# TissueImageAnalytics/cerberus

Measured on AMD Instinct MI355X. Metric: Mpx/sec WSI tiled inference (all heads), higher is better.
Workload: dtype f32

## Files before the change

### cerberus_amd/csrc/cerb_api.hip

```cpp
#include "cerb_net.h"

static thread_local std::string g_err;
int cerb_set_error(const std::string& m) {
    g_err = m;
    return 1;
}
extern "C" int cerb_version(void) { return 1; }
extern "C" const char* cerb_last_error(void) { return g_err.c_str(); }
std::atomic<long long> g_devbuf_bytes{0};
extern "C" size_t cerb_device_bytes_held(void) { const long long v = g_devbuf_bytes.load(); return v > 0 ? (size_t)v : 0; }
thread_local hipStream_t g_call_stream = nullptr;

static int alloc_dev(cerb_net* net, size_t bytes, void** out) {
    if (net->reusing) {
        if (net->reuse_cursor >= net->n_finalize_allocs || net->dev_alloc_bytes[net->reuse_cursor] != bytes)
            return fail("reload: the tensors do not have the shapes the handle was finalized with");
        *out = net->dev_allocs[net->reuse_cursor++];
        return 0;
    }
    void* d = nullptr;
    HIP_OK(hipMalloc(&d, bytes));
    net->dev_allocs.push_back(d);
    net->dev_alloc_bytes.push_back(bytes);
    *out = d;
// ... 366 lines not shown
        }
        for (int di : net->dense_idx) {
            const DecoderCfg& d = net->dec[di];
            const std::string p = "output_head." + d.name + "." + d.head + ".x";
            const HostTensor *w1, *b1, *w2, *b2;
            Fold f;
            if (get(net, p + ".0.block.0.conv.weight", {96, 64, 1, 1}, &w1) || get(net, p + ".0.block.0.conv.bias", {96}, &b1) ||
                bn_fold(net, p + ".0.block.0.bn", 96, &f) || get(net, p + ".1.conv.weight", {d.out_ch, 96, 1, 1}, &w2) ||
                get(net, p + ".1.conv.bias", {d.out_ch}, &b2))
                return 1;
            std::vector<float> w1p(6 * 4 * 64 * 4), b1p(96), w2p(6 * 64 * 4, 0.f), b2p(32, 0.f);
            for (int blk = 0; blk < 6; ++blk)
                for (int G = 0; G < 4; ++G)
                    for (int lane = 0; lane < 64; ++lane)
                        for (int t = 0; t < 4; ++t) {
                            const int hid = blk * 16 + (lane & 15), ci = G * 16 + 4 * (lane >> 4) + t;
                            w1p[((blk * 4 + G) * 64 + lane) * 4 + t] = w1->data[(size_t)hid * 64 + ci] * f.scale[hid];
                        }
            for (int c = 0; c < 96; ++c) b1p[c] = b1->data[c] * f.scale[c] + f.shift[c];
            for (int blk = 0; blk < 6; ++blk)
                for (int lane = 0; lane < 64; ++lane)
                    for (int r = 0; r < 4; ++r) {
                        const int o = lane & 15, hid = blk * 16 + 4 * (lane >> 4) + r;
                        w2p[(blk * 64 + lane) * 4 + r] = (o < d.out_ch) ? w2->data[(size_t)o * 96 + hid] : 0.f;
                    }
            for (int c = 0; c < d.out_ch; ++c) b2p[c] = b2->data[c];
            std::vector<float> w2q(2 * 24 * 64, 0.f);
            for (int set = 0; set < 2; ++set)
                for (int blk = 0; blk < 6; ++blk)
                    for (int r = 0; r < 4; ++r)
                        for (int lane = 0; lane < 64; ++lane) {
                            const int o = 4 * set + (lane & 3), hid = blk * 16 + 4 * (lane >> 4) + r;
                            if (o < d.out_ch) w2q[((set * 6 + blk) * 64 + lane) * 4 + r] = w2->data[(size_t)o * 96 + hid];
                        }
            if (!net->fold_bn) {
                float *r1, *rb1, *r2, *rb2;
                if (upload(net, w1->data, &r1) || upload(net, b1->data, &rb1) || upload(net, w2->data, &r2) || upload(net, b2->data, &rb2)) return 1;
                net->head_rw1.push_back(r1); net->head_rb1.push_back(rb1); net->head_rw2.push_back(r2); net->head_rb2.push_back(rb2);
                net->param_slots[p + ".0.block.0.conv.weight"].push_back({r1, 96 * 64});
                net->param_slots[p + ".0.block.0.conv.bias"].push_back({rb1, 96});
                net->param_slots[p + ".1.conv.weight"].push_back({r2, (long long)d.out_ch * 96});
                net->param_slots[p + ".1.conv.bias"].push_back({rb2, d.out_ch});
                if (store_bn(net, "head." + std::to_string(net->head_rw1.size() - 1), {p + ".0.block.0.bn"}, 96)) return 1;
            }
            float *dw1, *db1, *dw2, *db2;
            float* dw2q;
            if (upload(net, w1p, &dw1) || upload(net, b1p, &db1) || upload(net, w2p, &dw2) || upload(net, b2p, &db2) || upload(net, w2q, &dw2q)) return 1;
            net->head_w1.push_back(dw1); net->head_b1.push_back(db1); net->head_w2.push_back(dw2); net->head_b2.push_back(db2); net->head_w2q.push_back(dw2q);
        }
    }
    if (net->pc_idx >= 0) {
        const int oc = net->dec[net->pc_idx].out_ch;
        const std::string p = "decoder_head.Patch-Class";
        Fold f1, f2;
        const HostTensor *w1, *b1, *w2, *b2;
        if (bn_fold(net, p + ".bn1", 512, &f1) || bn_fold(net, p + ".bn2", 256, &f2) || get(net, p + ".conv1.weight", {256, 512, 1, 1}, &w1) ||
            get(net, p + ".conv1.bias", {256}, &b1) || get(net, p + ".conv2.weight", {oc, 256, 1, 1}, &w2) || get(net, p + ".conv2.bias", {oc}, &b2))
            return 1;
        if (!net->fold_bn) {
            if (upload(net, w1->data, &net->pc_rw1) || upload(net, b1->data, &net->pc_rb1) || upload(net, w2->data, &net->pc_rw2) ||
                upload(net, b2->data, &net->pc_rb2) || store_bn(net, "pc.bn1", {p + ".bn1"}, 512) || store_bn(net, "pc.bn2", {p + ".bn2"}, 256))
                return 1;
            net->param_slots[p + ".conv1.weight"].push_back({net->pc_rw1, 256 * 512});
            net->param_slots[p + ".conv1.bias"].push_back({net->pc_rb1, 256});
            net->param_slots[p + ".conv2.weight"].push_back({net->pc_rw2, (long long)oc * 256});
            net->param_slots[p + ".conv2.bias"].push_back({net->pc_rb2, oc});
        }
        std::vector<float> w1t(512 * 256), b1f(256), w2t(256 * 16, 0.f), b2f(16, 0.f);
        for (int o = 0; o < 256; ++o) {
            for (int c = 0; c < 512; ++c) w1t[(size_t)c * 256 + o] = w1->data[(size_t)o * 512 + c] * f2.scale[o];
            b1f[o] = b1->data[o] * f2.scale[o] + f2.shift[o];
        }
        for (int o = 0; o < oc; ++o) {
            for (int c = 0; c < 256; ++c) w2t[(size_t)c * 16 + o] = w2->data[(size_t)o * 256 + c];
            b2f[o] = b2->data[o];
        }
        if (upload(net, f1.scale, &net->pc_bn1s) || upload(net, f1.shift, &net->pc_bn1b) || upload(net, w1t, &net->pc_w1t) ||
            upload(net, b1f, &net->pc_b1) || upload(net, w2t, &net->pc_w2t) || upload(net, b2f, &net->pc_b2))
            return 1;
    }
    if (!net->fold_bn) {
        std::vector<float> z(512, 0.f);
        if (upload(net, z, &net->zero_bias)) return 1;
    }
    if (!net->fold_bn) HIP_OK(hipDeviceSynchronize());
    if (net->reusing && net->reuse_cursor != net->n_finalize_allocs) return fail("reload: fewer tensors than the handle was finalized with");
    if (!net->reusing) net->n_finalize_allocs = net->dev_allocs.size();
    net->reusing = false;
    net->host.clear();
    net->finalized = true;
    return 0;
}

int prof_begin(cerb_net* net, const std::string& name, const std::string& kernel, double flops, hipStream_t st) {
    if (!net->profiling) return 0;
    if (net->prof_n == net->prof.size()) {
        cerb_net::ProfRec r;
        HIP_OK(hipEventCreate(&r.e0));
        HIP_OK(hipEventCreate(&r.e1));
        net->prof.push_back(r);
    }
    cerb_net::ProfRec& r = net->prof[net->prof_n];
    r.name = name; r.kernel = kernel; r.flops = flops;
    HIP_OK(hipEventRecord(r.e0, st));
    net->prof_open = true;
    return 0;
}
int prof_end(cerb_net* net, hipStream_t st) {
    if (!net->profiling) return 0;
    HIP_OK(hipEventRecord(net->prof[net->prof_n].e1, st));
    net->prof_n++;
    net->prof_open = false;
    return 0;
}

int train_wino2_fresh(cerb_net* net, const std::string& name, PackedConv& cm, int dgrad, hipStream_t st) {
    if (net->fold_bn) return 0;
    bool& used = dgrad ? cm.wino_dgrad_used : cm.wino_used;
    bool& stale = dgrad ? cm.wino_dgrad_stale : cm.wino_stale;
    used = true;
    if (!stale) return 0;
    auto rit = net->raw.find(name);
    if (rit == net->raw.end()) return fail("conv " + name + ": no raw weights to re-pack");
    const size_t nw = (size_t)cm.cout * cm.cin * 9, nu = (size_t)cm.cout * cm.cin * 16;
    for (int g = 0; g < cm.groups; ++g)
        HIP_OK(cerb_launch_pack_wino(rit->second.w + g * nw, (dgrad ? cm.wino_dgrad : cm.wino) + g * nu, dgrad ? cm.cin : cm.cout, dgrad ? cm.cout : cm.cin, dgrad, st));
    stale = false;
    return 0;
}

int train_wino4_slot(cerb_net* net, const std::string& name, PackedConv& cm, int w4b, int dgrad, hipStream_t st, float** out) {
    float*& slot = cm.wino4_t[w4b][dgrad];
    if (!slot) {
        auto rit = net->raw.find(name);
        if (rit == net->raw.end()) return fail("conv " + name + ": no raw weights for the F(4x4) transform");
        const size_t nw = (size_t)cm.cout * cm.cin * 9, nu = (size_t)cm.cout * cm.cin * 36;
        void* d = nullptr;
        HIP_OK(hipMalloc(&d, (size_t)cm.groups * nu * 4));
        net->dev_allocs.push_back(d);
        net->dev_alloc_bytes.push_back((size_t)cm.groups * nu * 4);
        slot = (float*)d;
        (void)nw;
        HIP_OK(cerb_launch_pack_wino4(rit->second.w, slot, dgrad ? cm.cin : cm.cout, dgrad ? cm.cout : cm.cin, dgrad, w4b, cm.groups, st));
    }
    *out = slot;
    return 0;
}

static constexpr int kPlanarLowest = 0;
static const char* const kPlanarFamily[4] = {"conv_wino4_planar<f4x4,16x16x2,eighth-res>", "conv_wino4_planar<f4x4,16x16x2,quarter-res>",
                                             "conv_wino4p<f4x4,16x16x2,planar,half-res>", "conv_wino4p<f4x4,16x16x2,planar>"};
static const char* const kPlanarEntryFamily[4] = {"upsample2_add_planar<eighth-res>", "upsample2_add_planar<quarter-res>", "upsample2_add_planar", "upsample2_add_planar"};

int run_conv(cerb_net* net, const std::string& name, const float* in, const float* prev, const float* resid, float* out, int N,
             int H, int W, int relu, int mode, long long in_gs, long long prev_gs, hipStream_t st, double* macs,
             const int* roi, long long planar_out_gs) {
    auto it = net->conv.find(name);
    if (it == net->conv.end()) return fail("internal: conv " + name + " not packed");
    const PackedConv& c = it->second;
    struct BnReq {
        cerb_net* n;
        ~BnReq() { n->conv_bn_part = nullptr; }
    } bn_req{net};
    net->conv_bn_bpg = 0;
    ConvParams p;
    memset(&p, 0, sizeof(p));
    p.in = in; p.prev = prev; p.wpack = c.w; p.bias = c.b; p.resid = resid; p.out = out;
    p.N = N; p.H = H; p.W = W; p.Cin = c.cin; p.Cout = c.cout;
    p.Ho = (c.stride == 2) ? H / 2 : H;
    p.Wo = (c.stride == 2) ? W / 2 : W;
    p.relu = relu;
    p.groups = c.groups;
    p.in_gs = in_gs; p.prev_gs = prev_gs;
    p.w_gs = (long long)c.cout * c.cin * c.ks * c.ks;
    p.bias_gs = c.cout;
    p.resid_gs = 0;
    p.out_gs = (long long)N * p.Ho * p.Wo * c.cout;
    p.pk_off = net->packed_items ? 0 : 1;
    if (macs) {
        *macs += (double)c.groups * N * p.Ho * p.Wo * (double)c.cout * c.cin * c.ks * c.ks;
        if (!out) return 0;
    }
    const double fl = 2.0 * (double)c.groups * N * p.Ho * p.Wo * (double)c.cout * c.cin * c.ks * c.ks;
    const long long map_px = (long long)p.Ho * p.Wo;
    const bool use_w4 = net->conv_algo == 5 || net->conv_algo == 7 || (net->conv_algo == 6 && map_px >= 256);
    const bool planar = planar_out_gs > 0;
    static const long long w4b_max_px = [] {
        const char* e = cerb_dev_getenv("CERB_W4B_MAX_PX");
        return e ? atoll(e) : 4096ll;
    }();
    const bool w4b = !planar && (net->conv_algo == 7 || (net->conv_algo == 6 && map_px <= w4b_max_px)) && c.cin % 64 == 0;
    if (planar && !(use_w4 && c.wino && mode == 0 && net->fold_bn && !resid)) return fail("internal: conv " + name + " cannot take the planar path");
    if (use_w4 && c.wino && mode == 0 && (!it->second.host_w.empty() || !net->fold_bn)) {
        PackedConv& cm = it->second;
        float* train_slot = nullptr;
        if (!net->fold_bn && train_wino4_slot(net, name, cm, w4b ? 1 : 0, 0, st, &train_slot)) return 1;
        float*& slot4 = !net->fold_bn ? train_slot : (w4b ? cm.wino4b : cm.wino4);
        if (!slot4) {
            std::vector<float> w4;
            for (int g = 0; g < cm.groups; ++g) pack_wino4(cm.host_w.data() + (size_t)g * cm.cout * cm.cin * 9, cm.cout, cm.cin, &w4, w4b ? 1 : 0);
            void* d = nullptr;
            HIP_OK(hipMalloc(&d, w4.size() * 4));
            net->dev_allocs.push_back(d);
            net->dev_alloc_bytes.push_back(w4.size() * 4);
            HIP_OK(hipMemcpy(d, w4.data(), w4.size() * 4, hipMemcpyHostToDevice));
            slot4 = (float*)d;
        }
        p.wpack = slot4;
        p.w_gs = (long long)c.cout * c.cin * 36;
        double fl_done = fl;
        if (roi && roi[1] > roi[0] && roi[3] > roi[2]) {
            p.roi_y0 = roi[0]; p.roi_y1 = roi[1]; p.roi_x0 = roi[2]; p.roi_x1 = roi[3];
            const double ty = (roi[1] + 15) / 16 - roi[0] / 16, tx = (roi[3] + 15) / 16 - roi[2] / 16;
            fl_done = fl * (ty * 16.0 * tx * 16.0) / ((double)p.Ho * p.Wo);
        }
        if (planar) {
            p.out_gs = planar_out_gs;
            p.level_tag = net->planar_level == 3 ? 1 : net->planar_level == 2 ? 0 : 2;
            p.pl_byp = cerb_planar_blocks(p.Ho);
            p.pl_bxp = cerb_planar_blocks(p.Wo);
        }
        if (prof_begin(net, name, planar ? kPlanarFamily[net->planar_level & 3] : w4b ? (cerb_wino4b_packed(p) ? (resid ? "conv_wino4b<f4x4,16t,res>" : "conv_wino4b<f4x4,16t>") : (resid ? "conv_wino4b<f4x4,16x16,res>" : "conv_wino4b<f4x4,16x16>")) : (resid ? "conv_wino4<f4x4,16x16x2,res>" : "conv_wino4<f4x4,16x16x2>"), fl_done, st)) return 1;
        if (net->conv_bn_part && !planar && !resid && !(roi && roi[1] > roi[0] && roi[3] > roi[2])) {
            p.bn_part = net->conv_bn_part;
            net->conv_bn_bpg = w4b ? cerb_wino4b_bn_blocks(p) : N * ((p.Ho + 15) / 16) * ((p.Wo + 15) / 16);
        }
        HIP_OK(planar ? cerb_launch_wino4p(p, st) : w4b ? cerb_launch_wino4b(p, st) : cerb_launch_wino4(p, st));
        if (prof_end(net, st)) return 1;
        return 0;
    }
    if (net->conv_algo && c.wino && mode == 0) {
        if (train_wino2_fresh(net, name, it->second, 0, st)) return 1;
        p.wpack = c.wino;
        p.w_gs = (long long)c.cout * c.cin * 16;
        double fl_done = fl;
        if (roi && roi[1] > roi[0] && roi[3] > roi[2]) {
            p.roi_y0 = roi[0]; p.roi_y1 = roi[1]; p.roi_x0 = roi[2]; p.roi_x1 = roi[3];
            const double ty = (roi[1] + 7) / 8 - roi[0] / 8, tx = (roi[3] + 15) / 16 - roi[2] / 16;
            fl_done = fl * (ty * 8.0 * tx * 16.0) / ((double)p.Ho * p.Wo);
        }
        if (prof_begin(net, name, resid ? "conv_wino<f2x2,8x16,res>" : "conv_wino<f2x2,8x16>", fl_done, st)) return 1;
        HIP_OK(cerb_launch_wino(p, st));
        if (prof_end(net, st)) return 1;
        return 0;
    }
    const std::string kn = "conv_igemm<ks" + std::to_string(c.ks) + ",s" + std::to_string(c.stride) + ",mode" + std::to_string(mode) +
                           (p.Wo < 32 ? ",16x16>" : ",8x32>");
    if (prof_begin(net, name, kn, fl, st)) return 1;
    HIP_OK(cerb_launch_conv(p, c.ks, c.stride, mode, st));
    if (prof_end(net, st)) return 1;
    return 0;
}

static int forward_impl(cerb_net* net, const cerb_forward_io* io, hipStream_t st, double* macs) {
    g_call_stream = st;
    const bool dry = (macs != nullptr) && (io->tiles == nullptr) && (io->tiles_f32 == nullptr);
    const int N = io->n, H = io->h, W = io->w;
    if (N <= 0 || H <= 0 || W <= 0 || (H % 16) || (W % 16)) return fail("cerb_net_forward: tile H,W must be positive multiples of 16");
    const int out_h = io->out_h > 0 ? io->out_h : H, out_w = io->out_w > 0 ? io->out_w : W;
    if (out_h > H || out_w > W) return fail("cerb_net_forward: crop larger than tile");
    const int hs[5] = {H, H / 2, H / 4, H / 8, H / 16}, ws[5] = {W, W / 2, W / 4, W / 8, W / 16};
    const size_t D = net->trunk_idx.size();
    const size_t guard = cerb_conv_guard_bytes(W);
    const int planar_lowest = [] {
        const char* e = cerb_dev_getenv("CERB_PLANAR_LOWEST");
        return e ? atoi(e) : kPlanarLowest;
    }();
    auto level_is_planar = [&](int u) {
        if (dry || !net->planar || !net->fold_bn || net->conv_algo != 6 || net->head_algo < 1) return false;
        for (int v = 3; v >= u; --v) {
            if (v < planar_lowest) return false;
            auto c0 = net->conv.find("dec." + std::to_string(v) + ".0"), c1 = net->conv.find("dec." + std::to_string(v) + ".1");
            if (c0 == net->conv.end() || c1 == net->conv.end() || !c0->second.wino || !c1->second.wino) return false;
            const long long px = (long long)hs[3 - v] * ws[3 - v];
            if ((hs[3 - v] & 3) || (ws[3 - v] & 3)) return false;
            const bool ok = v >= 2 ? px >= 4096 && c0->second.cin == 64 && c0->second.cout == 64 && c1->second.cout == 64
                                   : px >= 256 && c0->second.cin % 16 == 0 && c0->second.cout % 64 == 0 && c1->second.cin == c0->second.cout && c1->second.cout % 64 == 0;
            if (!ok) return false;
        }
        return true;
    };
    if (!dry) {
        if (net->x0.ensure((size_t)N * H * W * 64 * 4, guard) || net->pool.ensure((size_t)N * hs[1] * ws[1] * 64 * 4, guard)) return fail_alloc();
        for (int i = 1; i < 5; ++i)
            if (net->x[i].ensure((size_t)N * hs[i] * ws[i] * kFilters[i] * 4, guard)) return fail_alloc();
        if (net->ta.ensure((size_t)N * hs[1] * ws[1] * 64 * 4, guard) || net->tb.ensure((size_t)N * hs[1] * ws[1] * 64 * 4, guard) ||
            net->cm.ensure((size_t)N * hs[4] * ws[4] * 256 * 4, guard))
            return fail_alloc();
        if (D) {
            static const bool exact_ws = cerb_dev_getenv("CERB_LEGACY_WS") == nullptr;
            size_t need_sum = 0, need_mid = 0;
            const int oc[4] = {128, 64, 64, 64};
            for (int u = 0; u < 4; ++u) {
                if (exact_ws && level_is_planar(u)) continue;
                const std::string n0 = "dec." + std::to_string(u) + ".0";
                auto c0 = net->conv.find(n0);
                const size_t px = (size_t)D * N * hs[3 - u] * ws[3 - u];
                need_sum = std::max(need_sum, px * (size_t)(c0 != net->conv.end() ? c0->second.cin : 256) * 4);
                need_mid = std::max(need_mid, px * (size_t)(c0 != net->conv.end() ? c0->second.cout : 256) * 4);
            }
            if (!exact_ws) need_sum = need_mid = D * (size_t)N * H * W * 64 * 4;
            if (net->dmid.ensure(need_mid, guard)) return fail_alloc();
            if (net->conv_algo && net->dsum.ensure(need_sum, guard)) return fail_alloc();
            for (int u = 0; u < 4; ++u) {
                if (exact_ws && level_is_planar(u)) continue;
                if (net->dout[u].ensure(D * (size_t)N * hs[3 - u] * ws[3 - u] * oc[u] * 4, guard)) return fail_alloc();
            }
        }
    }
    if (macs) *macs += (double)N * H * W * 64.0 * 147.0;
    if (!dry) {
        StemParams sp;
        sp.tiles = io->tiles; sp.tiles_f32 = io->tiles ? nullptr : io->tiles_f32; sp.wpack = net->stem_w; sp.bias = net->stem_b; sp.out = net->x0.p; sp.N = N; sp.H = H; sp.W = W; sp.relu = 1;
        sp.tiles_x = sp.tiles_y = 0;
        if (prof_begin(net, "stem", "stem_conv7x7", 2.0 * N * H * W * 64.0 * 147.0, st)) return 1;
        HIP_OK(cerb_launch_stem(sp, st));
        if (prof_end(net, st)) return 1;
        if (prof_begin(net, "maxpool", "maxpool3x3s2", 0.0, st)) return 1;
        HIP_OK(cerb_launch_maxpool(net->x0.p, net->pool.p, N, H, W, 64, st));
        if (prof_end(net, st)) return 1;
    }
    float* cur = dry ? nullptr : net->pool.p;
    int inpl = 64;
    for (int li = 0; li < 4; ++li) {
        const int planes = kFilters[li + 1];
        const int Hi = (li == 0) ? hs[1] : hs[li], Wi = (li == 0) ? ws[1] : ws[li];
        for (int b = 0; b < kLayers[li]; ++b) {
            const std::string p = "backbone.layer" + std::to_string(li + 1) + "." + std::to_string(b);
            const int stride = (b == 0 && li > 0) ? 2 : 1;
            const int hin = (b == 0) ? Hi : hs[li + 1], win = (b == 0) ? Wi : ws[li + 1];
            float* t1 = dry ? nullptr : net->ta.p;
            const bool last = (b == kLayers[li] - 1);
            float* outb = dry ? nullptr : (((kLayers[li] - 1 - b) % 2 == 0) ? net->x[li + 1].p : net->tb.p);
            (void)last;
            const float* idt = cur;
            if (run_conv(net, p + ".conv1", cur, nullptr, nullptr, t1, N, hin, win, 1, 0, 0, 0, st, macs)) return 1;
            if (stride != 1 || inpl != planes) {
                float* ds = dry ? nullptr : net->pool.p;
                if (run_conv(net, p + ".downsample", cur, nullptr, nullptr, ds, N, hin, win, 0, 0, 0, 0, st, macs)) return 1;
                idt = ds;
            }
            if (run_conv(net, p + ".conv2", t1, nullptr, idt, outb, N, hs[li + 1], ws[li + 1], 1, 0, 0, 0, st, macs)) return 1;
            cur = outb;
            inpl = planes;
        }
    }
    if (run_conv(net, "conv_map", dry ? nullptr : net->x[4].p, nullptr, nullptr, dry ? nullptr : net->cm.p, N, hs[4], ws[4], 0, 0, 0, 0, st, macs)) return 1;

    const long long tile_stride = io->tile_stride ? io->tile_stride : (long long)out_h * out_w;
    const long long row_stride = io->row_stride ? io->row_stride : out_w;
    if (net->pc_idx >= 0) {
        if (macs) *macs += (double)N * (512.0 * 256 + 256.0 * net->dec[net->pc_idx].out_ch);
        const bool want = io->out && io->out[net->pc_idx];
        const bool wantl = io->logits && io->logits[net->pc_idx];
        if (!dry && (want || wantl)) {
            PatchClassParams pp;
            memset(&pp, 0, sizeof(pp));
            pp.x4 = net->x[4].p; pp.bn1_s = net->pc_bn1s; pp.bn1_b = net->pc_bn1b; pp.w1t = net->pc_w1t; pp.b1 = net->pc_b1;
            pp.w2t = net->pc_w2t; pp.b2 = net->pc_b2;
            pp.N = N; pp.Hf = hs[4]; pp.Wf = ws[4]; pp.out_ch = net->dec[net->pc_idx].out_ch;
            pp.out_h = out_h; pp.out_w = out_w;
            pp.logits = wantl ? io->logits[net->pc_idx] : nullptr;
            pp.out = want ? (float*)io->out[net->pc_idx] : nullptr;
            pp.tile_off = io->tile_off; pp.tile_stride = tile_stride; pp.row_stride = row_stride;
            if (prof_begin(net, "patch_class", "patch_class", 2.0 * N * (512.0 * 256 + 256.0 * pp.out_ch), st)) return 1;
            HIP_OK(cerb_launch_patch_class(pp, st));
            if (prof_end(net, st)) return 1;
        }
    }
    if (D) {
        const float* skips[4] = {dry ? nullptr : net->x[3].p, dry ? nullptr : net->x[2].p, dry ? nullptr : net->x[1].p, dry ? nullptr : net->x0.p};
        const float* prev = dry ? nullptr : net->cm.p;
        long long prev_gs = 0;
        const int oc[4] = {128, 64, 64, 64};
        int roi_out[4][4], roi_mid[4][4], roi_sum[4][4];
        const bool any_logits = [&] {
            if (!io->logits) return false;
            for (size_t k = 0; k < net->dec.size(); ++k)
                if (io->logits[k]) return true;
            return false;
        }();
        const bool use_roi = !dry && net->crop_roi && (net->conv_algo == 1 || net->conv_algo >= 5) && !any_logits && (out_h < H || out_w < W);
        if (use_roi) {
            int y0 = (int)((H - out_h) * 0.5), x0 = (int)((W - out_w) * 0.5), y1 = y0 + out_h, x1 = x0 + out_w;
            for (int u = 3; u >= 0; --u) {
                const int hh = hs[3 - u], ww = ws[3 - u];
                auto widen = [&](int* r, const int* in, int d) {
                    r[0] = std::max(0, (in[0] - d) & ~3); r[1] = std::min(hh, (in[1] + d + 3) & ~3);
                    r[2] = std::max(0, (in[2] - d) & ~3); r[3] = std::min(ww, (in[3] + d + 3) & ~3);
                };
                const int win[4] = {y0, y1, x0, x1};
                widen(roi_out[u], win, 0);
                widen(roi_mid[u], roi_out[u], 1);
                widen(roi_sum[u], roi_mid[u], 1);
                y0 = std::max(0, roi_sum[u][0] / 2 - 1); y1 = std::min(hh / 2, (roi_sum[u][1] - 1) / 2 + 2);
                x0 = std::max(0, roi_sum[u][2] / 2 - 1); x1 = std::min(ww / 2, (roi_sum[u][3] - 1) / 2 + 2);
            }
        }
        bool feat_planar = false, prev_planar = false;
        for (int u = 0; u < 4; ++u) {
            const int hh = hs[3 - u], ww = ws[3 - u];
            const std::string n0 = "dec." + std::to_string(u) + ".0", n1 = "dec." + std::to_string(u) + ".1";
            const int cmid = net->conv[n0].cout;
            const int cin0 = net->conv[n0].cin;
            const bool lvl_planar = level_is_planar(u);
            if (lvl_planar) {
                PlanarBuf &bs = u == 3 ? net->psum : u == 2 ? net->psum2 : u == 1 ? net->psum1 : net->psum0;
                PlanarBuf &bm = u == 3 ? net->pmid : u == 2 ? net->pmid2 : u == 1 ? net->pmid1 : net->pmid0;
                const int cout1 = net->conv[n1].cout;
                PlanarBuf& bo = cout1 == cin0 ? bs : u == 1 ? net->pout1 : net->pout0;
                if (bs.ensure((int)D, N, hh, ww, cin0, st) || bm.ensure((int)D, N, hh, ww, cmid, st) || (&bo != &bs && bo.ensure((int)D, N, hh, ww, cout1, st)))
                    return fail_alloc();
                if (prof_begin(net, n0 + ".up", kPlanarEntryFamily[u], 0.0, st)) return 1;
                HIP_OK(cerb_launch_upsample2_add_planar(skips[u], prev, bs.b.p, (int)D, N, hh, ww, cin0, prev_gs, bs.gs(), use_roi ? roi_sum[u] : nullptr, prev_planar ? 1 : 0, st));
                if (prof_end(net, st)) return 1;
                net->planar_level = u;
                if (run_conv(net, n0, bs.b.p, nullptr, nullptr, bm.b.p, N, hh, ww, 1, 0, bs.gs(), 0, st, macs, use_roi ? roi_mid[u] : nullptr, bm.gs()))
                    return 1;
                if (run_conv(net, n1, bm.b.p, nullptr, nullptr, bo.b.p, N, hh, ww, 1, 0, bm.gs(), 0, st, macs, use_roi ? roi_out[u] : nullptr, bo.gs()))
                    return 1;
                if (u == 3) feat_planar = true;
                prev = bo.b.p;
                prev_gs = bo.gs();
                prev_planar = true;
                continue;
            }
            if (prev_planar) return fail("internal: a tile-planar decoder level feeds an NHWC one");
            if (net->conv_algo && net->conv[n0].wino && !dry) {
                if (prof_begin(net, n0 + ".up", "upsample2_add", 0.0, st)) return 1;
                HIP_OK(cerb_launch_upsample2_add(skips[u], prev, net->dsum.p, (int)D, N, hh, ww, cin0, prev_gs, use_roi ? roi_sum[u] : nullptr, st));
                if (prof_end(net, st)) return 1;
                if (run_conv(net, n0, net->dsum.p, nullptr, nullptr, net->dmid.p, N, hh, ww, 1, 0, (long long)N * hh * ww * cin0, 0, st, macs,
                             use_roi ? roi_mid[u] : nullptr))
                    return 1;
            } else if (run_conv(net, n0, skips[u], prev, nullptr, dry ? nullptr : net->dmid.p, N, hh, ww, 1, 1, 0, prev_gs, st, macs)) return 1;
            if (run_conv(net, n1, dry ? nullptr : net->dmid.p, nullptr, nullptr, dry ? nullptr : net->dout[u].p, N, hh, ww, 1, 0,
                         (long long)N * hh * ww * cmid, 0, st, macs, use_roi ? roi_out[u] : nullptr))
                return 1;
            prev = dry ? nullptr : net->dout[u].p;
            prev_gs = (long long)N * hh * ww * oc[u];
        }
        HeadParams hps[8];
        int n_hp = 0;
        double head_flops = 0.0;
        for (size_t k = 0; k < net->dense_idx.size(); ++k) {
            const int di = net->dense_idx[k];
            const size_t tk = (size_t)net->trunk_of[k];
            const DecoderCfg& d = net->dec[di];
            if (macs) *macs += (double)N * H * W * (64.0 * 96 + 96.0 * d.out_ch);
            const bool want = io->out && io->out[di];
            const bool wantl = io->logits && io->logits[di];
            if (dry || !(want || wantl)) continue;
            HeadParams hp;
            memset(&hp, 0, sizeof(hp));
            hp.feat = feat_planar ? net->psum.b.p + tk * net->psum.gs() : net->dout[3].p + tk * (size_t)N * H * W * 64;
            hp.feat_planar = feat_planar ? 1 : 0;
            hp.pl_byp = cerb_planar_blocks(H);
            hp.pl_bxp = cerb_planar_blocks(W);
            hp.w1p = net->head_w1[k]; hp.b1 = net->head_b1[k]; hp.w2p = net->head_w2[k]; hp.b2 = net->head_b2[k]; hp.w2q = net->head_w2q[k];
            hp.N = N; hp.H = H; hp.W = W; hp.out_ch = d.out_ch; hp.kind = d.kind;
            hp.crop_y0 = (int)((H - out_h) * 0.5); hp.crop_x0 = (int)((W - out_w) * 0.5);
            hp.out_h = want ? out_h : 0; hp.out_w = want ? out_w : 0;
            hp.roi = use_roi ? 1 : 0;
            hp.logits = wantl ? io->logits[di] : nullptr;
            hp.absmax_bits = io->logit_absmax ? io->logit_absmax + di : nullptr;
            if (want) {
                if (d.kind == 0) hp.out_inst = (float*)io->out[di];
                else if (io->type_is_u8) hp.out_type_u8 = (unsigned char*)io->out[di];
                else hp.out_type_i64 = (long long*)io->out[di];
            }
            hp.tile_off = io->tile_off; hp.tile_stride = tile_stride; hp.row_stride = row_stride;
            const double head_px = hp.roi ? (double)out_h * (((hp.crop_x0 + out_w + 15) / 16 - hp.crop_x0 / 16) * 16.0) : (double)H * W;
            const double fl = 2.0 * N * head_px * (64.0 * 96 + 96.0 * d.out_ch);
            if (net->head_algo == 0) {
                if (prof_begin(net, "head." + d.name, "head", fl, st)) return 1;
                HIP_OK(cerb_launch_head(hp, st));
                if (prof_end(net, st)) return 1;
            } else {
                if (n_hp == 8) {
// ... 231 lines not shown
```

### cerberus_amd/csrc/cerb_net.h

```cpp
#ifndef CERB_NET_H
#define CERB_NET_H
#include <hip/hip_runtime.h>

#include <algorithm>
#include <cmath>
#include <cstdio>
#include <cstdlib>
#include <cstring>
#include <map>
#include <atomic>
#include <string>
#include <vector>

#include "../../include/cerberus_hip.h"
#include "cerb_common.h"

hipError_t cerb_launch_conv(const ConvParams& p, int ks, int stride, int mode, hipStream_t st);
hipError_t cerb_launch_wino(ConvParams p, hipStream_t st);
hipError_t cerb_launch_wino4(ConvParams p, hipStream_t st);
hipError_t cerb_launch_wino4b(ConvParams p, hipStream_t st);
int cerb_wino4b_bn_blocks(const ConvParams& p);
bool cerb_wino4b_packed(const ConvParams& p);
hipError_t cerb_launch_wino4p(ConvParams p, hipStream_t st);
hipError_t cerb_launch_upsample2_add_planar(const float* skip, const float* prev, float* out, int groups, int N, int H, int W, int C, long long prev_gs,
                                            long long out_gs, const int* roi, int prev_planar, hipStream_t st);
hipError_t cerb_launch_upsample2_add(const float* skip, const float* prev, float* out, int groups, int N, int H, int W, int C,
                                     long long prev_gs, const int* roi, hipStream_t st);
extern "C" int cerb_conv_chunk(int ks, int stride);
struct StemParams {
    const unsigned char* tiles;
    const float* tiles_f32;
    const float* wpack;
    const float* bias;
    float* out;
    int N, H, W, tiles_x, tiles_y;
    int relu;
};
hipError_t cerb_launch_stem(StemParams p, hipStream_t st);
size_t cerb_bn_workspace_bytes(int groups, long long rows, int C);
hipError_t cerb_launch_bn_stats(const float* x, long long group_stride, long long rows, int C, int groups, float eps, float* mean, float* rstd,
                                float* var_unbiased, void* ws, hipStream_t st);
hipError_t cerb_launch_bn_apply(float* x, const float* src, const float* resid, long long group_stride, long long rows, int C, int groups, const float* mean,
                                const float* rstd, const float* gamma, const float* beta, int relu, hipStream_t st);
hipError_t cerb_launch_bn_finalize(const double* partial, int blocks, long long rows, int C, float eps, float* mean, float* rstd, float* var_unbiased, hipStream_t st,
                                   int groups = 1, void* fold_ws = nullptr);
size_t cerb_bn_fold_workspace_bytes(int groups, int C);
hipError_t cerb_launch_pointwise(const float* in, const float* w, const float* bias, float* out, long long rows, int cin, int cout, const float* in_scale,
                                 hipStream_t st, double* bn_part = nullptr, int* bn_blocks = nullptr);
hipError_t cerb_launch_crop_gap(const float* x, int N, int H, int W, int C, int y0, int ch, int x0, int cw, float* out, hipStream_t st);
hipError_t cerb_launch_copy_multi(int count, float* const* dst, const float* const* src, const long long* n, void** dev_tab, size_t* dev_bytes,
                                  std::vector<char>* host_prev, hipStream_t st);
hipError_t cerb_launch_bn_bwd(const float* dz, const float* z, const float* y, float* dy, float* dresid, long long group_stride, long long rows, int C, int groups,
                              const float* mean, const float* rstd, const float* gamma, const float* beta, float* dgamma, float* dbeta, int relu, int dy_assign, void* ws, hipStream_t st, unsigned long long eval_mask = 0, int dresid_assign = 0,
                              const double* pre_part = nullptr, int pre_bpg = 0);
int cerb_head_bwd2_blocks();
hipError_t cerb_launch_conv_bwd(const float* x, const float* dy, const float* w, float* dx, float* dw, float* db, int G, int N, int H, int W, int Cin, int Cout,
                                int ks, int stride, long long x_gs, hipStream_t st);
hipError_t cerb_launch_stem_wgrad(const unsigned char* tiles, const float* dy, float* dw, int N, int H, int W, hipStream_t st);
hipError_t cerb_launch_maxpool_bwd(const float* x, const float* ypool, const float* dy, float* dx, int N, int H, int W, int C, hipStream_t st);
hipError_t cerb_launch_maxpool_idx(const float* in, float* out, unsigned* idx, int N, int H, int W, int C, hipStream_t st);
hipError_t cerb_launch_maxpool_bwd_idx(const unsigned* idx, const float* dy, float* dx, int N, int H, int W, int C, hipStream_t st);
bool cerb_upadd_bwd_fused_ok(int H, int W, int C, int G);
hipError_t cerb_launch_upadd_bwd(const float* dout, float* dskip, float* dprev, int G, int N, int H, int W, int C, long long prev_gs, int shared_prev, hipStream_t st,
                                 unsigned group_mask = 0xffffffffu, int skip_assign = 0, int prev_assign = 0);
hipError_t cerb_launch_pointwise_bwd(const float* x, const float* dy, const float* w, float* dx, float* dw, float* db, long long rows, int cin, int cout,
                                     const float* in_scale, int dx_assign, hipStream_t st);
hipError_t cerb_launch_crop_gap_bwd(const float* dg, float* dx, int N, int H, int W, int C, int y0, int ch, int x0, int cw, hipStream_t st);
hipError_t cerb_launch_adam(float* p, const float* g, float* m, float* v, long long n, float lr, float b1, float b2, float eps, int step, hipStream_t st);
size_t cerb_wgrad_workspace_bytes(int G, int N, int Ho, int Wo, int Cin, int Cout, int ks, int* slices_out);
size_t cerb_stem_wgrad_workspace_bytes();
hipError_t cerb_launch_pack_stem(const float* w_raw, float* out, hipStream_t st);
struct PackJob {
    const float* w;
    float* out;
    long long total;
    int cout, cin, kind, a, b, pad;
};
hipError_t cerb_launch_pack_multi(const PackJob* jobs, int count, void** dev_tab, size_t* dev_bytes, std::vector<char>* host_prev, hipStream_t st);
hipError_t cerb_launch_adam_multi(int count, float* const* p, const float* const* g, float* const* m, float* const* v, const long long* n, float lr, float b1,
                                  float b2, float eps, int step, hipStream_t st);
hipError_t cerb_launch_pack_conv(const float* w_raw, float* out, int cout, int cin, int ks, int chunk, hipStream_t st);
hipError_t cerb_launch_pack_wino(const float* w_raw, float* out, int cout, int cin, int dgrad, hipStream_t st);
hipError_t cerb_launch_pack_wino4(const float* w_raw, float* out, int cout, int cin, int dgrad, int chunk32, int groups, hipStream_t st);
hipError_t cerb_launch_dilate2(const float* dy, float* d, long long n, int H, int W, int C, hipStream_t st);
size_t cerb_pw_wgrad_small_workspace_bytes(long long rows, int cin, int cout);
hipError_t cerb_launch_pw_wgrad_small(const float* x, const float* dy, float* dw, long long rows, int cin, int cout, void* ws, hipStream_t st);
size_t cerb_pw_bwd_small_workspace_bytes(long long rows, int cin, int cout);
hipError_t cerb_launch_pw_bwd_small(const float* x, const float* dy, const float* w, float* dx, float* dw, float* db, long long rows, int cin, int cout,
                                    int dx_assign, void* ws, hipStream_t st);
hipError_t cerb_launch_stem_wgrad_mfma(const unsigned char* tiles, const float* dy, float* dw, int N, int H, int W, void* ws, hipStream_t st);
hipError_t cerb_launch_colsum(const float* d, long long group_stride, long long rows, int C, int G, float* out, void* ws, hipStream_t st);
bool cerb_wgrad_wino_supported(int H, int W, int Cin, int Cout);
size_t cerb_wgrad_wino_workspace_bytes(int G, int N, int H, int W, int Cin, int Cout);
hipError_t cerb_launch_wgrad_wino(const float* x, const float* dy, float* dw, int G, int N, int H, int W, int Cin, int Cout, long long x_gs, void* ws, hipStream_t st,
                                  float* db);
hipError_t cerb_launch_wgrad(const float* x, const float* dy, float* dw, int G, int N, int H, int W, int Cin, int Cout, int ks, int stride, long long x_gs, void* ws,
                             hipStream_t st, float* db = nullptr);
bool cerb_head_train_supported(long long rows, int cin, int chid, int out);
hipError_t cerb_launch_head_fwd1(const float* prev, const float* w1, const float* b1, float* hid, long long rows, double* bn_part, int* bn_blocks, hipStream_t st,
                                 const float* const* in_bn = nullptr);
hipError_t cerb_launch_head_fwd2(const float* hid, const float* mean, const float* rstd, const float* gamma, const float* beta, const float* w2, const float* b2,
                                 float* logits, long long rows, int out, hipStream_t st);
size_t cerb_head_bwd_workspace_bytes(long long rows, int out);
hipError_t cerb_launch_head_bwd1(const float* hid, const float* dlog, const float* mean, const float* rstd, const float* gamma, const float* beta, const float* w2,
                                 float* dw2, float* db2, float* dgamma, float* dbeta, long long rows, int out, void* ws, hipStream_t st);
hipError_t cerb_launch_head_bwd2(const float* hid, const float* dlog, const float* prev, const float* mean, const float* rstd, const float* gamma, const float* beta,
                                 const float* dgamma, const float* dbeta, const float* w1, const float* w2, float* dprev, float* dw1, float* db1, long long rows, int out,
                                 int eval_mode, int assign, void* ws, hipStream_t st, const float* const* in_bn = nullptr, double* in_part = nullptr);
hipError_t cerb_launch_maxpool(const float* in, float* out, int N, int H, int W, int C, hipStream_t st);
hipError_t cerb_launch_head(const HeadParams& p, hipStream_t st);
hipError_t cerb_launch_head_group(const HeadParams* heads, int n_heads, hipStream_t st, int w2_44);
struct PatchClassParams {
    const float* x4;
    const float* bn1_s;
    const float* bn1_b;
    const float* w1t;
    const float* b1;
    const float* w2t;
    const float* b2;
    int N, Hf, Wf, out_ch;
    int out_h, out_w;
    float* logits;
    float* out;
    const long long* tile_off;
    long long tile_stride, row_stride;
};
hipError_t cerb_launch_patch_class(const PatchClassParams& p, hipStream_t st);

int cerb_set_error(const std::string& m);
static inline int fail(const std::string& m) { return cerb_set_error(m); }
static inline int fail_alloc() { return cerb_set_error("workspace allocation failed") + 1; }
#define HIP_OK(expr)                                                                              \
    do {                                                                                          \
        hipError_t e_ = (expr);                                                                   \
        if (e_ != hipSuccess) return fail(std::string(#expr) + ": " + hipGetErrorString(e_));     \
    } while (0)

struct HostTensor {
    std::vector<int64_t> shape;
    std::vector<float> data;
};

extern "C" size_t cerb_conv_guard_bytes(int tile_w);
extern thread_local hipStream_t g_call_stream;
extern std::atomic<long long> g_devbuf_bytes;
struct DevBuf {
    float* p = nullptr;
    char* raw = nullptr;
    size_t bytes = 0, guard = 0, held = 0;
    int ensure(size_t need, size_t g) {
        if (need <= bytes && g <= guard) return 0;
        release();
        if (hipMalloc(&raw, need + 2 * g) != hipSuccess) {
            raw = nullptr;
            return 1;
        }
        g_devbuf_bytes += (long long)(need + 2 * g);
        held = need + 2 * g;
        if (hipMemsetAsync(raw, 0, need + 2 * g, g_call_stream) != hipSuccess) return 1;
        p = reinterpret_cast<float*>(raw + g);
        bytes = need;
        guard = g;
        return 0;
    }
    void release() {
        if (raw) {
            (void)hipFree(raw);
            g_devbuf_bytes -= (long long)held;
        }
        held = 0;
        raw = nullptr;
        p = nullptr;
        bytes = guard = 0;
    }
};

struct PlanarBuf {
    DevBuf b;
    int h = 0, w = 0, c = 0, groups = 0;
    long long cap_n = 0;
    long long per_image() const { return cerb_planar_elems(1, h, w, c); }
    long long gs() const { return cap_n * per_image(); }
    int ensure(int G, int N, int H, int W, int C, hipStream_t st) {
        if (H == h && W == w && C == c && G == groups && N <= cap_n) return 0;
        const size_t need = (size_t)G * (size_t)N * (size_t)cerb_planar_elems(1, H, W, C) * 4;
        if (need > b.bytes) {
            if (b.ensure(need, 0)) return 1;
        } else if (hipMemsetAsync(b.raw, 0, b.bytes + 2 * b.guard, st) != hipSuccess) {
            return 1;
        }
        h = H; w = W; c = C; groups = G;
        cap_n = (long long)(b.bytes / ((size_t)G * (size_t)cerb_planar_elems(1, H, W, C) * 4));
        return 0;
    }
    void release() { b.release(); h = w = c = groups = 0; cap_n = 0; }
};

struct PackedConv {
    int cin = 0, cout = 0, ks = 0, stride = 1, groups = 1;
    float* w = nullptr;
    float* wino = nullptr;
    float* wino_dgrad = nullptr;
    bool wino_used = false, wino_dgrad_used = false, wino_stale = false, wino_dgrad_stale = false;
    float* wino4_t[2][2] = {{nullptr, nullptr}, {nullptr, nullptr}};
    float* wino4b = nullptr;
    float* wino4 = nullptr;
    std::vector<float> host_w;
    float* b = nullptr;
};

struct DecoderCfg {
    std::string name, head;
    int out_ch = 0;
    int kind = 0;
};

struct cerb_net {
    std::vector<DecoderCfg> dec;
    std::vector<int> dense_idx;
    std::vector<int> trunk_idx;
    std::vector<int> trunk_of;
    int pc_idx = -1;
    std::map<std::string, HostTensor> host;
    bool finalized = false;
    float *stem_w = nullptr, *stem_b = nullptr;
    std::map<std::string, PackedConv> conv;
    std::vector<float*> head_w1, head_b1, head_w2, head_b2, head_w2q;
    float *pc_bn1s = nullptr, *pc_bn1b = nullptr, *pc_w1t = nullptr, *pc_b1 = nullptr, *pc_w2t = nullptr, *pc_b2 = nullptr;
    std::vector<void*> dev_allocs;
    std::vector<size_t> dev_alloc_bytes;
    size_t n_finalize_allocs = 0, reuse_cursor = 0;
    bool reusing = false;
    int fold_bn = 1;
    struct BnDev {
        float *gamma = nullptr, *beta = nullptr;
        int C = 0, groups = 1;
        float *run_mean = nullptr, *run_rstd = nullptr;
        std::vector<char> eval;
    };
    std::map<std::string, BnDev> bn;
    std::vector<float*> head_rw1, head_rb1, head_rw2, head_rb2;
    float *pc_rw1 = nullptr, *pc_rb1 = nullptr, *pc_rw2 = nullptr, *pc_rb2 = nullptr;
    DevBuf t_mean, t_rstd, t_ws, t_hid, t_gap, t_pc1, t_idn, t_dil;
    struct RawW { float* w = nullptr; float* b = nullptr; std::vector<std::string> wkeys, bkeys, bnkeys; };
    std::map<std::string, RawW> raw;
    struct ParamSlot { float* dst; long long n; };
    std::map<std::string, std::vector<ParamSlot>> param_slots;
    float* stem_raw = nullptr;
    std::vector<DevBuf> tape;
    size_t tape_pos = 0;
    void* copy_tab = nullptr;
    size_t copy_tab_bytes = 0;
    std::vector<char> copy_tab_host;
    void* pack_tab = nullptr;
    size_t pack_tab_bytes = 0;
    std::vector<char> pack_tab_host;
    float* zero_bias = nullptr;
    std::map<std::string, std::pair<float*, long long>> grads;
    std::map<std::string, std::vector<std::string>> bn_keys;
    DevBuf x0, pool, x[5], ta, tb, cm, dmid, dsum, dout[4];
    PlanarBuf psum, pmid, pout;
    int planar_level = 3;
    PlanarBuf psum2, pmid2, pout2;
    PlanarBuf psum1, pmid1, pout1, psum0, pmid0, pout0;
    int packed_items = 1;
    int planar = 1;
    bool profiling = false;
    int crop_roi = 1;
    int head_algo = 1;
    int conv_algo = 6;
    struct ProfRec { std::string name, kernel; double flops; hipEvent_t e0, e1; };
    std::vector<ProfRec> prof;
    size_t prof_n = 0;
    bool prof_open = false;
    double* conv_bn_part = nullptr;
    int conv_bn_bpg = 0;
    hipStream_t side = nullptr;
    hipEvent_t ev_fork = nullptr, ev_join = nullptr;
    DevBuf t_ws2;
    ~cerb_net() {
        if (side) { (void)hipStreamSynchronize(side); (void)hipStreamDestroy(side); }
        if (ev_fork) (void)hipEventDestroy(ev_fork);
        if (ev_join) (void)hipEventDestroy(ev_join);
        t_ws2.release();
        for (auto& r : prof) { (void)hipEventDestroy(r.e0); (void)hipEventDestroy(r.e1); }
        for (void* p : dev_allocs) (void)hipFree(p);
        if (copy_tab) (void)hipFree(copy_tab);
        if (pack_tab) (void)hipFree(pack_tab);
        x0.release(); pool.release(); ta.release(); tb.release(); cm.release(); dmid.release(); dsum.release(); psum.release(); pmid.release(); pout.release(); psum2.release(); pmid2.release(); pout2.release(); psum1.release(); pmid1.release(); pout1.release(); psum0.release(); pmid0.release(); pout0.release();
        t_mean.release(); t_rstd.release(); t_ws.release(); t_hid.release(); t_gap.release(); t_pc1.release(); t_idn.release(); t_dil.release();
        for (auto& b : tape) b.release();
        for (auto& b : x) b.release();
        for (auto& b : dout) b.release();
    }
};


static const int kLayers[4] = {3, 4, 6, 3};
static const int kFilters[5] = {64, 64, 128, 256, 512};
int prof_begin(cerb_net* net, const std::string& name, const std::string& kernel, double flops, hipStream_t st);
int prof_end(cerb_net* net, hipStream_t st);
int train_wino2_fresh(cerb_net* net, const std::string& name, PackedConv& cm, int dgrad, hipStream_t st);
int train_wino4_slot(cerb_net* net, const std::string& name, PackedConv& cm, int w4b, int dgrad, hipStream_t st, float** out);
int run_conv(cerb_net* net, const std::string& name, const float* in, const float* prev, const float* resid, float* out, int N, int H, int W, int relu, int mode,
             long long in_gs, long long prev_gs, hipStream_t st, double* macs, const int* roi = nullptr, long long planar_out_gs = 0);
#endif
```

### cerberus_amd/csrc/conv_igemm.hip

```cpp
#include "wino_common.h"

__device__ __forceinline__ f32x4 splat4(float x) {
    f32x4 r = {x, x, x, x};
    return r;
}

template <int KS, int STRIDE, int TH, int TW, int CB, int MODE>
struct ConvCfg {
    static constexpr int PAD = KS / 2;
    static constexpr int GSTEP = (KS == 1) ? STRIDE : 1;
    static constexpr int LSTEP = (KS == 1) ? 1 : STRIDE;
    static constexpr int IH = (KS == 1) ? TH : (TH - 1) * STRIDE + KS;
    static constexpr int IW = (KS == 1) ? TW : (TW - 1) * STRIDE + KS;
    static constexpr int PS = CB + 4;
    static constexpr int NG = CB / 8;
    static constexpr int T = KS * KS;
    static constexpr int NQ = T * NG;
    static constexpr int PARTS = CB / 4;
    static constexpr int PPS = 256 / PARTS;
    static constexpr int NF = IH * IW * PARTS;
    static constexpr int RPS = 32 / TW;
    static constexpr int NM = (IH + RPS - 1) / RPS;
    static constexpr int NE = (2 * IH * 8 + 255) / 256;
    static constexpr int ITER = (MODE == 1) ? NM + NE : (NF + 255) / 256;
    static constexpr int MAIN_FLOATS = IH * IW * PS;
    static constexpr int AR = TH / 2 + 2, AC = TW / 2 + 2;
    static constexpr int NA = AR * AC * PARTS;
    static constexpr int AITER = (NA + 255) / 256;
    static constexpr int AUX_FLOATS = (MODE == 1) ? AR * AC * PS : 0;
    static constexpr int LDS_FLOATS = MAIN_FLOATS + AUX_FLOATS;
    static constexpr int LDS_BYTES = LDS_FLOATS * 4;
    static constexpr int S_PREV = ITER;
    static constexpr int S_BAR = ITER + AITER + 6;
    static constexpr int S_COMB = S_BAR + 1;
    static constexpr int WD = (MODE == 0 && STRIDE == 1) ? 3 : 2;
};

struct Item {
    int g, cb, n, oy0, ox0, tx, ty;
};

template <int KS, int STRIDE, int TH, int TW, int CB, int MODE>
__global__ __launch_bounds__(256, 2) void conv_igemm_kernel(ConvParams p) {
    using C = ConvCfg<KS, STRIDE, TH, TW, CB, MODE>;
    constexpr int WD = C::WD;
    static_assert(TH * TW == 256, "tile must hold 256 pixels (4 waves x 2 x 32)");
    static_assert(MODE == 0 || (KS == 3 && STRIDE == 1 && CB == 32 && C::IH % C::RPS == 0 && C::S_COMB + C::ITER <= C::NQ),
                  "MODE 1 schedule must fit in one chunk");
    static_assert(C::ITER <= 2 * C::NQ || KS == 1, "every staging slice needs a step");
    extern __shared__ __attribute__((aligned(16))) float lds[];

    const int tid = threadIdx.x;
    const int lane = tid & 63;
    const int wave = tid >> 6;
    const int j = lane & 31;
    const int h = lane >> 5;

    const int ncb = p.Cout >> 6;
    const int ntile = p.N * p.tiles_y * p.tiles_x;
    const int per_group = ntile * ncb;
    const int total = per_group * p.groups;
    const int nchunk = p.Cin / CB;
    const int lb = xcd_remap(blockIdx.x, gridDim.x);
    const int base_cnt = total / (int)gridDim.x, rem_cnt = total % (int)gridDim.x;
    int item = lb * base_cnt + min(lb, rem_cnt);
    const int item_end = item + base_cnt + (lb < rem_cnt ? 1 : 0);
    if (item >= item_end) return;

    auto decode = [&](int it) {
        Item w;
        w.g = it / per_group;
        int L = it - w.g * per_group;
        w.cb = L % ncb;
        int t_ = L / ncb;
        w.tx = t_ % p.tiles_x;
        t_ /= p.tiles_x;
        w.ty = t_ % p.tiles_y;
        w.n = t_ / p.tiles_y;
        w.oy0 = w.ty * TH;
        w.ox0 = w.tx * TW;
        return w;
    };
    auto advance = [&](Item w) {
        if (++w.cb == ncb) {
            w.cb = 0;
            if (++w.tx == p.tiles_x) {
                w.tx = 0;
                if (++w.ty == p.tiles_y) {
                    w.ty = 0;
                    if (++w.n == p.N) {
                        w.n = 0;
                        ++w.g;
                    }
                }
            }
        }
        w.oy0 = w.ty * TH;
        w.ox0 = w.tx * TW;
        return w;
    };
    auto in_base = [&](const Item& w) {
        return reinterpret_cast<const char*>(p.in + w.g * p.in_gs) +
               ((((long long)w.n * p.H + (w.oy0 * STRIDE - C::PAD)) * p.W + (w.ox0 * STRIDE - C::PAD)) * p.Cin) * 4;
    };
    auto w_base = [&](const Item& w) {
        return reinterpret_cast<const char*>(p.wpack + w.g * p.w_gs + (long long)w.cb * nchunk * C::NQ * 2 * 256);
    };
    auto touches_border = [&](const Item& w) {
        const int y0 = w.oy0 * STRIDE - C::PAD, x0 = w.ox0 * STRIDE - C::PAD;
        return y0 < 0 || x0 < 0 || y0 + (C::IH - 1) * C::GSTEP + 1 > p.H || x0 + (C::IW - 1) * C::GSTEP + 1 > p.W;
    };

    constexpr int RPS = C::RPS, NM = C::NM, NE = C::NE;
    unsigned soff[MODE == 1 ? 1 + NE : C::ITER];
    int ldsw0, ldswE = 0;
    bool e_last_ok = true;
    const int rowb = p.W * p.Cin * 4;
    if (MODE == 1) {
        const int mrow = (tid >> 3) / TW, mcol = (tid >> 3) % TW, part = tid & 7;
        soff[0] = (unsigned)(((mrow * p.W + mcol) * p.Cin + part * 4) * 4);
        ldsw0 = (mrow * C::IW + mcol) * C::PS + part * 4;
        const int e_iy = tid >> 4, e_ix = TW + ((tid >> 3) & 1);
#pragma unroll
        for (int k = 0; k < NE; ++k) {
            const int iy = min(e_iy + 16 * k, C::IH - 1);
            soff[1 + k] = (unsigned)(((iy * p.W + e_ix) * p.Cin + part * 4) * 4);
        }
        ldswE = (e_iy * C::IW + e_ix) * C::PS + part * 4;
        e_last_ok = e_iy + 16 * (NE - 1) < C::IH;
    } else {
#pragma unroll
        for (int s = 0; s < C::ITER; ++s) {
            const int f = min(tid + s * 256, C::NF - 1);
            const int pix = f / C::PARTS, part = f % C::PARTS;
            soff[s] = (unsigned)((((pix / C::IW) * C::GSTEP * p.W + (pix % C::IW) * C::GSTEP) * p.Cin + part * 4) * 4);
        }
        ldsw0 = (tid / C::PARTS) * C::PS + (tid % C::PARTS) * 4;
    }
    const unsigned wlane = (unsigned)lane * 16u;
    int ldsb[2];
    unsigned ooff[2];
#pragma unroll
    for (int q = 0; q < 2; ++q) {
        const int pl = (wave * 2 + q) * 32 + j;
        const int py = pl / TW, px = pl % TW;
        ldsb[q] = ((py * C::LSTEP) * C::IW + px * C::LSTEP) * C::PS + 4 * h;
        ooff[q] = (unsigned)(((py * p.Wo + px) * p.Cout + 4 * h) * 4);
    }
    float* aux = lds + C::MAIN_FLOATS;
    int aoffM = 0, aoffE[NE];
    float wM[4] = {0.f, 0.f, 0.f, 0.f}, wE[4] = {0.f, 0.f, 0.f, 0.f};
    int auxw0 = 0;
    if (MODE == 1) {
        const int mrow = (tid >> 3) / TW, mcol = (tid >> 3) % TW, part = tid & 7;
        aoffM = (mcol >> 1) * C::PS + part * 4;
        const float lxM = (mcol & 1) ? 0.75f : 0.25f;
        const float lyM = (RPS == 2 && (mrow & 1)) ? 0.75f : 0.25f;
        wM[0] = (1.f - lyM) * (1.f - lxM), wM[1] = (1.f - lyM) * lxM, wM[2] = lyM * (1.f - lxM), wM[3] = lyM * lxM;
        const int e_iy = tid >> 4, e_b = (tid >> 3) & 1;
#pragma unroll
        for (int k = 0; k < NE; ++k) aoffE[k] = ((min(e_iy + 16 * k, C::IH - 1) >> 1) * C::AC + TW / 2) * C::PS + part * 4;
        const float lxE = e_b ? 0.75f : 0.25f, lyE = (e_iy & 1) ? 0.75f : 0.25f;
        wE[0] = (1.f - lyE) * (1.f - lxE), wE[1] = (1.f - lyE) * lxE, wE[2] = lyE * (1.f - lxE), wE[3] = lyE * lxE;
        auxw0 = (tid / C::PARTS) * C::PS + (tid % C::PARTS) * 4;
    }

    f32x4 v[C::ITER];
    f32x4 pvv[C::AITER > 0 ? C::AITER : 1];
    unsigned poff[MODE == 1 ? C::AITER : 1];

    auto issue = [&](__amdgpu_buffer_rsrc_t r, int chunk_off, int s) {
        if (MODE == 1) {
            if (s < NM) v[s] = buf_load(r, soff[0], chunk_off + s * RPS * rowb);
            else v[s] = buf_load(r, soff[1 + s - NM], chunk_off);
        } else {
            v[s] = buf_load(r, soff[s], chunk_off);
        }
    };
    auto prev_offsets = [&](const Item& w) {
        const int Hp = p.H >> 1, Wp = p.W >> 1;
#pragma unroll
        for (int k = 0; k < C::AITER; ++k) {
            const int f = min(tid + k * 256, C::NA - 1);
            const int apix = f / C::PARTS, part = f % C::PARTS;
            const int py = min(max((w.oy0 >> 1) - 1 + apix / C::AC, 0), Hp - 1), px = min(max((w.ox0 >> 1) - 1 + apix % C::AC, 0), Wp - 1);
            poff[k] = (unsigned)(((py * Wp + px) * p.Cin + part * 4) * 4);
        }
    };
    auto prev_base = [&](const Item& w) {
        return reinterpret_cast<const char*>(p.prev + w.g * p.prev_gs + (long long)w.n * (p.H >> 1) * (p.W >> 1) * p.Cin);
    };
    auto write_prev = [&]() {
#pragma unroll
        for (int k = 0; k < C::AITER; ++k)
            if (tid + k * 256 < C::NA) *reinterpret_cast<f32x4*>(aux + auxw0 + k * C::PPS * C::PS) = pvv[k];
    };
    auto combine = [&](int s) {
        const bool main = s < NM;
        const float* a = main ? aux + aoffM + ((s * RPS) >> 1) * C::AC * C::PS : aux + aoffE[main ? 0 : s - NM];
        const f32x4 p00 = *reinterpret_cast<const f32x4*>(a);
        const f32x4 p01 = *reinterpret_cast<const f32x4*>(a + C::PS);
        const f32x4 p10 = *reinterpret_cast<const f32x4*>(a + C::AC * C::PS);
        const f32x4 p11 = *reinterpret_cast<const f32x4*>(a + C::AC * C::PS + C::PS);
        const bool swap = main && RPS == 1 && (s & 1);
        const float* wt = main ? wM : wE;
        f32x4 r = v[s];
        r = __builtin_elementwise_fma(splat4(wt[swap ? 2 : 0]), p00, r);
        r = __builtin_elementwise_fma(splat4(wt[swap ? 3 : 1]), p01, r);
        r = __builtin_elementwise_fma(splat4(wt[swap ? 0 : 2]), p10, r);
        r = __builtin_elementwise_fma(splat4(wt[swap ? 1 : 3]), p11, r);
        v[s] = r;
    };
    auto slice_iy = [&](int s) { return MODE == 1 ? (s < NM ? s * RPS + (tid >> 3) / TW : (tid >> 4) + 16 * (s - NM)) : ((tid + s * 256) / C::PARTS) / C::IW; };
    auto slice_ix = [&](int s) { return MODE == 1 ? (s < NM ? (tid >> 3) % TW : TW + ((tid >> 3) & 1)) : ((tid + s * 256) / C::PARTS) % C::IW; };
    auto slice_ptr = [&](int s) { return MODE == 1 ? (s < NM ? lds + ldsw0 + s * RPS * C::IW * C::PS : lds + ldswE + (s - NM) * 16 * C::IW * C::PS) : lds + ldsw0 + s * C::PPS * C::PS; };
    auto slice_live = [&](int s) { return MODE == 1 ? (s < C::ITER - 1 || e_last_ok) : (tid + s * 256 < C::NF); };
    auto write_tile = [&](const Item& w, bool masked) {
        if (!masked) {
#pragma unroll
            for (int s = 0; s < C::ITER; ++s)
                if (slice_live(s)) *reinterpret_cast<f32x4*>(slice_ptr(s)) = v[s];
        } else {
#pragma unroll
            for (int s = 0; s < C::ITER; ++s) {
                const int gy = w.oy0 * STRIDE - C::PAD + slice_iy(s) * C::GSTEP, gx = w.ox0 * STRIDE - C::PAD + slice_ix(s) * C::GSTEP;
                const bool ok = gy >= 0 && gy < p.H && gx >= 0 && gx < p.W;
                const f32x4 z = {0.f, 0.f, 0.f, 0.f};
                if (slice_live(s)) *reinterpret_cast<f32x4*>(slice_ptr(s)) = ok ? v[s] : z;
            }
        }
    };

    Item w = decode(item);
    {
        const __amdgpu_buffer_rsrc_t r0 = make_rsrc(in_base(w));
#pragma unroll
        for (int s = 0; s < C::ITER; ++s) issue(r0, 0, s);
    }
    if (MODE == 1) {
        prev_offsets(w);
        const __amdgpu_buffer_rsrc_t rp = make_rsrc(prev_base(w));
#pragma unroll
        for (int k = 0; k < C::AITER; ++k) pvv[k] = buf_load(rp, poff[k], 0);
        write_prev();
        __syncthreads();
#pragma unroll
        for (int s = 0; s < C::ITER; ++s) combine(s);
    }
    __amdgpu_buffer_rsrc_t rw = make_rsrc(w_base(w));
    f32x4 wq[WD + 1][2];
#pragma unroll
    for (int d = 0; d < WD; ++d)
#pragma unroll
        for (int s = 0; s < 2; ++s) wq[d][s] = buf_load(rw, wlane, (d * 2 + s) * 1024);

    for (;;) {
        f32x16 acc[2][2];
#pragma unroll
        for (int s = 0; s < 2; ++s)
#pragma unroll
            for (int q = 0; q < 2; ++q)
#pragma unroll
                for (int r = 0; r < 16; ++r) acc[s][q][r] = 0.f;

        const bool more_items = item + 1 < item_end;
        const Item wnx = more_items ? advance(w) : w;
        const __amdgpu_buffer_rsrc_t rw_nx = more_items ? make_rsrc(w_base(wnx)) : rw;
        const bool mask_cur = touches_border(w);

        for (int ch = 0; ch < nchunk; ++ch) {
            __syncthreads();
            write_tile(w, mask_cur);
            __syncthreads();

            const bool last_ch = (ch == nchunk - 1);
            const Item wp_ = last_ch ? wnx : w;
            const int chp = last_ch ? 0 : ch + 1;
            const __amdgpu_buffer_rsrc_t r_stage = make_rsrc(in_base(wp_));
            const int stage_off = chp * (CB * 4);
            __amdgpu_buffer_rsrc_t r_prev = r_stage;
            if (MODE == 1) {
                r_prev = make_rsrc(prev_base(wp_));
                if (last_ch) prev_offsets(wp_);
            }
            const int wcur_off = ch * (C::NQ * 2048);
            const __amdgpu_buffer_rsrc_t rw_over = last_ch ? rw_nx : rw;
            const int wover_off = last_ch ? 0 : (ch + 1) * (C::NQ * 2048);

            f32x4 b0 = *reinterpret_cast<const f32x4*>(lds + ldsb[0]), b1 = *reinterpret_cast<const f32x4*>(lds + ldsb[1]);
            f32x4 bn0 = b0, bn1 = b1;
#pragma unroll
            for (int tap = 0; tap < C::T; ++tap) {
#pragma unroll
                for (int G = 0; G < C::NG; ++G) {
                    const int q = tap * C::NG + G;
                    {
                        if (q + WD < C::NQ) {
                            wq[WD][0] = buf_load(rw, wlane, wcur_off + ((q + WD) * 2 + 0) * 1024);
                            wq[WD][1] = buf_load(rw, wlane, wcur_off + ((q + WD) * 2 + 1) * 1024);
                        } else {
                            wq[WD][0] = buf_load(rw_over, wlane, wover_off + ((q + WD - C::NQ) * 2 + 0) * 1024);
                            wq[WD][1] = buf_load(rw_over, wlane, wover_off + ((q + WD - C::NQ) * 2 + 1) * 1024);
                        }
                        if (q + 1 < C::NQ) {
                            const int tap1 = (q + 1) / C::NG, G1 = (q + 1) % C::NG;
                            const int toff1 = ((tap1 / KS) * C::IW + (tap1 % KS)) * C::PS + G1 * 8;
                            bn0 = *reinterpret_cast<const f32x4*>(lds + ldsb[0] + toff1);
                            bn1 = *reinterpret_cast<const f32x4*>(lds + ldsb[1] + toff1);
                        }
                    }
#pragma unroll
                    for (int s = q; s < C::ITER; s += C::NQ) issue(r_stage, stage_off, s);
                    if (MODE == 1) {
                        if (q >= C::S_PREV && q < C::S_PREV + C::AITER) pvv[q - C::S_PREV] = buf_load(r_prev, poff[q - C::S_PREV], stage_off);
                        if (q == C::S_BAR) {
                            write_prev();
                            __syncthreads();
                        }
                        if (q >= C::S_COMB && q - C::S_COMB < C::ITER) combine(q - C::S_COMB);
                    }
                    __builtin_amdgcn_sched_barrier(0);
#pragma unroll
                    for (int t = 0; t < 4; ++t) {
                        acc[0][0] = __builtin_amdgcn_mfma_f32_32x32x2f32(wq[0][0][t], b0[t], acc[0][0], 0, 0, 0);
                        acc[1][0] = __builtin_amdgcn_mfma_f32_32x32x2f32(wq[0][1][t], b0[t], acc[1][0], 0, 0, 0);
                        acc[0][1] = __builtin_amdgcn_mfma_f32_32x32x2f32(wq[0][0][t], b1[t], acc[0][1], 0, 0, 0);
                        acc[1][1] = __builtin_amdgcn_mfma_f32_32x32x2f32(wq[0][1][t], b1[t], acc[1][1], 0, 0, 0);
                    }
#pragma unroll
                    for (int d = 0; d < WD; ++d) {
                        wq[d][0] = wq[d + 1][0];
                        wq[d][1] = wq[d + 1][1];
                    }
                    b0 = bn0;
                    b1 = bn1;
                }
            }
        }

        {
            const float* bias = p.bias + w.g * p.bias_gs + w.cb * 64 + h * 4;
            const long long origin = (((long long)w.n * p.Ho + w.oy0) * p.Wo + w.ox0) * p.Cout + w.cb * 64;
            const __amdgpu_buffer_rsrc_t r_out = make_rsrc(p.out + w.g * p.out_gs + origin);
            const __amdgpu_buffer_rsrc_t r_res = make_rsrc(p.resid ? p.resid + w.g * p.resid_gs + origin : p.out);
            const bool has_res = p.resid != nullptr;
            const bool partial = (w.oy0 + TH > p.Ho) || (w.ox0 + TW > p.Wo);
#pragma unroll
            for (int q = 0; q < 2; ++q) {
                if (partial) {
                    const int pl = (wave * 2 + q) * 32 + j;
                    if (w.oy0 + pl / TW >= p.Ho || w.ox0 + pl % TW >= p.Wo) continue;
                }
#pragma unroll
                for (int s = 0; s < 2; ++s) {
#pragma unroll
                    for (int rq = 0; rq < 4; ++rq) {
                        const int co = s * 32 + rq * 8;
                        f32x4 o = {acc[s][q][rq * 4 + 0], acc[s][q][rq * 4 + 1], acc[s][q][rq * 4 + 2], acc[s][q][rq * 4 + 3]};
                        o = o + *reinterpret_cast<const f32x4*>(bias + co);
                        if (has_res) o = o + buf_load(r_res, ooff[q], co * 4);
                        if (p.relu) {
                            o[0] = fmaxf(o[0], 0.f);
                            o[1] = fmaxf(o[1], 0.f);
                            o[2] = fmaxf(o[2], 0.f);
                            o[3] = fmaxf(o[3], 0.f);
                        }
                        buf_store(o, r_out, ooff[q], co * 4);
                    }
                }
            }
        }
        if (!more_items) break;
        ++item;
        w = wnx;
        rw = rw_nx;
    }
}

template <int KS, int STRIDE, int TH, int TW, int CB, int MODE>
static hipError_t launch_cfg(ConvParams p, hipStream_t st) {
    using C = ConvCfg<KS, STRIDE, TH, TW, CB, MODE>;
    p.tiles_x = (p.Wo + TW - 1) / TW;
    p.tiles_y = (p.Ho + TH - 1) / TH;
    const long long items = (long long)p.groups * p.N * p.tiles_x * p.tiles_y * (p.Cout / 64);
    auto kern = conv_igemm_kernel<KS, STRIDE, TH, TW, CB, MODE>;
    static bool attr_done[64] = {};
    if (cerb_attr_needed(attr_done)) {
        hipError_t e = hipFuncSetAttribute(reinterpret_cast<const void*>(kern), hipFuncAttributeMaxDynamicSharedMemorySize, C::LDS_BYTES);
        if (e != hipSuccess) return e;
    }
    const int blocks_per_cu = (C::LDS_BYTES * 2 <= 160 * 1024) ? 2 : 1;
    long long grid = 256ll * blocks_per_cu;
    if (grid > items) grid = items;
    hipLaunchKernelGGL(kern, dim3((unsigned)grid), dim3(256), C::LDS_BYTES, st, p);
    return hipGetLastError();
}

extern "C" int cerb_conv_chunk(int ks, int stride) { return (stride == 2) ? 16 : 32; }

extern "C" size_t cerb_conv_guard_bytes(int tile_w) { return (size_t)17 * (size_t)tile_w * 64 * 4 + (64u << 10); }

hipError_t cerb_launch_conv(const ConvParams& p, int ks, int stride, int mode, hipStream_t st) {
    const bool small = p.Wo < 32;
    if (ks == 3 && stride == 1 && mode == 0) return small ? launch_cfg<3, 1, 16, 16, 32, 0>(p, st) : launch_cfg<3, 1, 8, 32, 32, 0>(p, st);
    if (ks == 3 && stride == 1 && mode == 1) return small ? launch_cfg<3, 1, 16, 16, 32, 1>(p, st) : launch_cfg<3, 1, 8, 32, 32, 1>(p, st);
    if (ks == 3 && stride == 2 && mode == 0) return small ? launch_cfg<3, 2, 16, 16, 16, 0>(p, st) : launch_cfg<3, 2, 8, 32, 16, 0>(p, st);
    if (ks == 1 && stride == 1 && mode == 0) return small ? launch_cfg<1, 1, 16, 16, 32, 0>(p, st) : launch_cfg<1, 1, 8, 32, 32, 0>(p, st);
    if (ks == 1 && stride == 2 && mode == 0) return small ? launch_cfg<1, 2, 16, 16, 16, 0>(p, st) : launch_cfg<1, 2, 8, 32, 16, 0>(p, st);
    return hipErrorInvalidValue;
}
```

### cerberus_amd/csrc/conv_wino4p.hip

```cpp
#include <type_traits>

#include "wino_common.h"

namespace {
constexpr int NPOS = 36;
constexpr int NT = 32;
constexpr int CB = 16;
constexpr int V_FLOATS = NPOS * NT * CB;
constexpr int LDS_BYTES = 2 * V_FLOATS * 4;
constexpr int PLANE_BYTES = 16 * 16 * 16 * 4;
constexpr int NS = NPOS;
constexpr int NPOS_A = 32;
#ifndef P4_RING
#define P4_RING 12
#endif
constexpr int RING = P4_RING;
#ifndef P4_WD
#define P4_WD 8
#endif
constexpr int WD = P4_WD;
#ifndef P4_PRE
#define P4_PRE P4_WD
#endif
constexpr int PRE = P4_PRE;
#ifndef P4_WB
#define P4_WB 1
#endif
constexpr int WB = P4_WB;
#ifndef P4_TQ
#define P4_TQ 22
#endif
constexpr int TQ = P4_TQ;
#ifndef P4_HQ
#define P4_HQ 8
#endif
constexpr int HQ = P4_HQ;
constexpr int halo_r(int k) { return k < 6 ? k : k < 14 ? ((k - 6) & 1 ? 5 : 0) : k - 14; }
constexpr int halo_q(int k) { return k < 6 ? 0 : k < 14 ? 1 + (k - 6) / 2 : 5; }
static_assert(NS % RING == 0 && WD + WB <= RING && NS % WB == 0 && PRE == WD && PRE <= RING, "weight ring");
static_assert(HQ + 10 <= TQ && TQ + 13 < NS && TQ + 8 + 4 <= NS, "the halo must be requested before the transform starts, the interior after its registers are free");
constexpr int BIAS_XI = 7;
constexpr int CHUNK_W_BYTES = NPOS * 4 * 1024;
constexpr int WAVE_W_BYTES = NPOS * 1024;

#ifdef P4_PROF
constexpr int PROF_BYTES = 16 * 40 * 8;
__device__ unsigned long long p4_prof_buf[16 * 40];
#ifndef P4_PROF_WAVE
#define P4_PROF_WAVE 0
#endif
#else
#ifdef P4_ABL_LDSPATCH
constexpr int PROF_BYTES = 16 * 1024;
#else
constexpr int PROF_BYTES = 0;
#endif
#endif

template <int I>
using IC = std::integral_constant<int, I>;
template <int B, int E, class F>
__device__ __forceinline__ void static_for(F&& f) {
    if constexpr (B < E) {
        f(IC<B>{});
        static_for<B + 1, E>(f);
    }
}

#ifndef P4_WAUX
#define P4_WAUX 0
#endif
#ifndef P4_PAUX
#define P4_PAUX 0
#endif

template <bool AGPR, bool ZERO>
__device__ __forceinline__ void mfma_step(f32x4& c0, f32x4& c1, const f32x4& av, const f32x4& b0, const f32x4& b1) {
#define P4_STEP_BODY(FIRST0, FIRST1)                               \
    "v_mfma_f32_16x16x4_f32 %0, %2, %6, " FIRST0 "\n\t"             \
    "v_mfma_f32_16x16x4_f32 %1, %2, %10, " FIRST1 "\n\t"            \
    "v_mfma_f32_16x16x4_f32 %0, %3, %7, %0\n\t"                     \
    "v_mfma_f32_16x16x4_f32 %1, %3, %11, %1\n\t"                    \
    "v_mfma_f32_16x16x4_f32 %0, %4, %8, %0\n\t"                     \
    "v_mfma_f32_16x16x4_f32 %1, %4, %12, %1\n\t"                    \
    "v_mfma_f32_16x16x4_f32 %0, %5, %9, %0\n\t"                     \
    "v_mfma_f32_16x16x4_f32 %1, %5, %13, %1"
#define P4_STEP_IN "v"(av[0]), "v"(av[1]), "v"(av[2]), "v"(av[3]), "v"(b0[0]), "v"(b0[1]), "v"(b0[2]), "v"(b0[3]), "v"(b1[0]), "v"(b1[1]), "v"(b1[2]), "v"(b1[3])
    if constexpr (ZERO) {
        if constexpr (AGPR) asm volatile(P4_STEP_BODY("0", "0") : "=&a"(c0), "=&a"(c1) : P4_STEP_IN);
        else asm volatile(P4_STEP_BODY("0", "0") : "=&v"(c0), "=&v"(c1) : P4_STEP_IN);
    } else {
        if constexpr (AGPR) asm volatile(P4_STEP_BODY("%0", "%1") : "+a"(c0), "+a"(c1) : P4_STEP_IN);
        else asm volatile(P4_STEP_BODY("%0", "%1") : "+v"(c0), "+v"(c1) : P4_STEP_IN);
    }
#undef P4_STEP_BODY
#undef P4_STEP_IN
}
#ifndef P4_ILV
#define P4_ILV 0
#endif
template <bool AGPR, bool ZERO>
__device__ __forceinline__ void mfma_pair(f32x4& c0, f32x4& c1, float a, float b0, float b1) {
    if constexpr (ZERO) {
        if constexpr (AGPR) asm volatile("v_mfma_f32_16x16x4_f32 %0, %2, %3, 0\n\tv_mfma_f32_16x16x4_f32 %1, %2, %4, 0" : "=&a"(c0), "=&a"(c1) : "v"(a), "v"(b0), "v"(b1));
        else asm volatile("v_mfma_f32_16x16x4_f32 %0, %2, %3, 0\n\tv_mfma_f32_16x16x4_f32 %1, %2, %4, 0" : "=&v"(c0), "=&v"(c1) : "v"(a), "v"(b0), "v"(b1));
    } else {
        if constexpr (AGPR) asm volatile("v_mfma_f32_16x16x4_f32 %0, %2, %3, %0\n\tv_mfma_f32_16x16x4_f32 %1, %2, %4, %1" : "+a"(c0), "+a"(c1) : "v"(a), "v"(b0), "v"(b1));
        else asm volatile("v_mfma_f32_16x16x4_f32 %0, %2, %3, %0\n\tv_mfma_f32_16x16x4_f32 %1, %2, %4, %1" : "+v"(c0), "+v"(c1) : "v"(a), "v"(b0), "v"(b1));
    }
}
__device__ __forceinline__ void wait_mfma_results() { asm volatile("s_nop 15\n\ts_nop 3"); }

__device__ __forceinline__ int fresh_lane() {
    int l;
    asm volatile("v_mbcnt_lo_u32_b32 %0, -1, 0\n\tv_mbcnt_hi_u32_b32 %0, -1, %0" : "=v"(l));
    return l;
}

__device__ __forceinline__ f32x4 sub4(const f32x4& x, const f32x4& y) {
    f32x2 lo, hi;
    const f32x2 xl = {x[0], x[1]}, xh = {x[2], x[3]}, yl = {y[0], y[1]}, yh = {y[2], y[3]};
    asm("v_pk_add_f32 %0, %1, %2 neg_lo:[0,1] neg_hi:[0,1]" : "=v"(lo) : "v"(xl), "v"(yl));
    asm("v_pk_add_f32 %0, %1, %2 neg_lo:[0,1] neg_hi:[0,1]" : "=v"(hi) : "v"(xh), "v"(yh));
    return f32x4{lo[0], lo[1], hi[0], hi[1]};
}

struct Blk {
    int n, by, bx;
};
struct Item {
    int g, cb;
    Blk b0, b1;
    int nvalid;
};
}

template <int LEVEL>
__global__ __launch_bounds__(256) __attribute__((amdgpu_waves_per_eu(1, 1))) void conv_wino4p_kernel(ConvParams p) {
    extern __shared__ __attribute__((aligned(16))) float lds[];
    const int tid = threadIdx.x;
    const int lane = tid & 63;
    const int a = __builtin_amdgcn_readfirstlane(tid >> 6);
    const int m = lane & 15;
    const int ks = lane >> 4;

    const int ncb = p.Cout >> 6;
    const int nblk = p.N * p.tiles_y * p.tiles_x;
    const int npair = (nblk + 1) >> 1;
    const int per_group = npair * ncb;
    const int total = per_group * p.groups;
    const int nchunk = p.Cin / CB;
    const int nplane_o = p.Cout / CB;
    const int lb = xcd_remap(blockIdx.x, gridDim.x);
    const int ISTEP = (int)gridDim.x;
    int item = lb;
    const int item_end = total;
    if (item >= item_end) return;
#ifdef P4_PROF
    const int prof_item = item + 2 * ISTEP;
#endif

    auto decode_blk = [&](int id) {
        Blk b;
        b.bx = id % p.tiles_x;
        const int r = id / p.tiles_x;
        b.by = r % p.tiles_y;
        b.n = r / p.tiles_y;
        return b;
    };
    auto decode = [&](int it) {
        Item w;
        w.g = it / per_group;
        const int L = it - w.g * per_group;
        w.cb = L % ncb;
        const int pr = L / ncb;
        w.nvalid = (2 * pr + 1 < nblk) ? 2 : 1;
        w.b0 = decode_blk(2 * pr);
        w.b1 = w.nvalid == 2 ? decode_blk(2 * pr + 1) : w.b0;
        return w;
    };
    auto in_base = [&](int g, const Blk& b) {
#ifdef P4_ABL_PATCHL2
        return reinterpret_cast<const char*>(p.in) + (((long long)(b.by & 1)) * p.pl_bxp + (b.bx & 3)) * (long long)nchunk * PLANE_BYTES;
#endif
        return reinterpret_cast<const char*>(p.in + g * p.in_gs) +
               (((long long)b.n * p.pl_byp + (b.by + p.ty_off)) * p.pl_bxp + (b.bx + p.tx_off)) * (long long)nchunk * PLANE_BYTES;
    };
    auto w_base = [&](const Item& w) {
        return reinterpret_cast<const char*>(p.wpack + w.g * p.w_gs) + (long long)w.cb * nchunk * CHUNK_W_BYTES + a * WAVE_W_BYTES;
    };

    const int t = tid >> 3, c = tid & 7, tm = t & 15, tty = tm >> 2, ttx = tm & 3;
    const bool second = (a >> 1) != 0;
    auto mine = [&](const Item& wi) {
        Blk b;
        b.n = second ? wi.b1.n : wi.b0.n;
        b.by = second ? wi.b1.by : wi.b0.by;
        b.bx = second ? wi.b1.bx : wi.b0.bx;
        return b;
    };
    unsigned poff[3][3];
    {
        const unsigned rowblk = (unsigned)p.pl_bxp * (unsigned)nchunk * PLANE_BYTES, colblk = (unsigned)nchunk * PLANE_BYTES;
#pragma unroll
        for (int rc = 0; rc < 3; ++rc)
#pragma unroll
            for (int qc = 0; qc < 3; ++qc) {
                const int dby = (rc == 0 && tty == 0) ? 0 : (rc == 2 && tty == 3) ? 2 : 1;
                const int dbx = (qc == 0 && ttx == 0) ? 0 : (qc == 2 && ttx == 3) ? 2 : 1;
                const int ty2 = rc == 0 ? ((tty + 3) & 3) : rc == 2 ? ((tty + 1) & 3) : tty;
                const int tx2 = qc == 0 ? ((ttx + 3) & 3) : qc == 2 ? ((ttx + 1) & 3) : ttx;
                poff[rc][qc] = (unsigned)dby * rowblk + (unsigned)dbx * colblk + (unsigned)((4 * ty2 + tx2) * 64 + c * 8);
                asm volatile("" : "+v"(poff[rc][qc]));
            }
    }
    const int vw = t * CB + (((c >> 1) ^ ((tm & 8) ? 3 : 0)) << 2) + 2 * (c & 1);
    const int vr = m * CB + ((ks ^ ((m & 8) ? 3 : 0)) << 2);
    const unsigned wlane = (unsigned)lane * 16u;

    f32x2 d[6][6];
#ifdef P4_ABL_PREVADD
    f32x2 pv[4][4];
#endif
    auto issue = [&](__amdgpu_buffer_rsrc_t r, int chunk_off, int rr, int qq) __attribute__((always_inline)) {
        const int ii = rr == 0 ? 3 : rr == 5 ? 0 : rr - 1, jj = qq == 0 ? 3 : qq == 5 ? 0 : qq - 1;
#ifdef P4_ABL_PREVADD
        if ((rr == 0 || rr == 1 || rr == 3 || rr == 5) && (qq == 0 || qq == 1 || qq == 3 || qq == 5))
            pv[rr == 0 ? 0 : rr == 1 ? 1 : rr == 3 ? 2 : 3][qq == 0 ? 0 : qq == 1 ? 1 : qq == 3 ? 2 : 3] =
                buf_load2<P4_PAUX>(r, poff[rr == 0 ? 0 : rr == 5 ? 2 : 1][qq == 0 ? 0 : qq == 5 ? 2 : 1], chunk_off + ((ii ^ 1) * 4 + (jj ^ 2)) * 1024);
#endif
#ifdef P4_ABL_LDSPATCH
        d[rr][qq] = *reinterpret_cast<const f32x2*>(lds + (rr * 6 + qq) * NT * CB + vw);
        return;
#endif
#ifdef P4_ABL_NOCORNER
        if ((rr == 0 || rr == 5) && (qq == 0 || qq == 5)) return;
#endif
#ifdef P4_ABL_NOEDGE
        if (rr == 0 || rr == 5 || qq == 0 || qq == 5) return;
#endif
#ifdef P4_ABL_HALOOWN
        d[rr][qq] = buf_load2<P4_PAUX>(r, poff[1][1], chunk_off + (ii * 4 + jj) * 1024);
        return;
#endif
#ifdef P4_ABL_CORNEROWN
        if ((rr == 0 || rr == 5) && (qq == 0 || qq == 5)) { d[rr][qq] = buf_load2<P4_PAUX>(r, poff[1][1], chunk_off + (ii * 4 + jj) * 1024); return; }
#endif
        d[rr][qq] = buf_load2<P4_PAUX>(r, poff[rr == 0 ? 0 : rr == 5 ? 2 : 1][qq == 0 ? 0 : qq == 5 ? 2 : 1], chunk_off + (ii * 4 + jj) * 1024);
    };
    f32x2 k2 = {2.f, 2.f}, k4 = {4.f, 4.f}, k5 = {5.f, 5.f};
    asm volatile("" : "+v"(k2), "+v"(k4), "+v"(k5));
#if defined(P4_ABL_PREVADD) && P4_ABL_PREVADD + 0 == 2
    f32x2 k75 = {0.75f, 0.75f}, k25 = {0.25f, 0.25f};
    asm volatile("" : "+v"(k75), "+v"(k25));
    auto blend = [&](const f32x2& wa, const f32x2& x, const f32x2& wb, const f32x2& y) __attribute__((always_inline)) {
        f32x2 t, r;
        asm("v_pk_mul_f32 %0, %1, %2" : "=v"(t) : "v"(wb), "v"(y));
        asm("v_pk_fma_f32 %0, %1, %2, %3" : "=v"(r) : "v"(wa), "v"(x), "v"(t));
        return r;
    };
    auto pass_v = [&](int q) __attribute__((always_inline)) {
        const int qa = q <= 1 ? 0 : q <= 3 ? 1 : 2, qb = qa + 1;
        const bool odd = (q & 1) != 0;
        f32x2 h[4];
#pragma unroll
        for (int r = 0; r < 4; ++r) h[r] = odd ? blend(k75, pv[r][qa], k25, pv[r][qb]) : blend(k25, pv[r][qa], k75, pv[r][qb]);
        const f32x2 v0 = blend(k25, h[0], k75, h[1]), v1 = blend(k75, h[1], k25, h[2]), v2 = blend(k25, h[1], k75, h[2]);
        const f32x2 v3 = blend(k75, h[2], k25, h[3]), v4 = blend(k25, h[2], k75, h[3]), v5 = blend(k75, h[2], k25, h[3]);
        asm("v_pk_add_f32 %0, %0, %1" : "+v"(d[0][q]) : "v"(v0));
        asm("v_pk_add_f32 %0, %0, %1" : "+v"(d[1][q]) : "v"(v1));
        asm("v_pk_add_f32 %0, %0, %1" : "+v"(d[2][q]) : "v"(v2));
        asm("v_pk_add_f32 %0, %0, %1" : "+v"(d[3][q]) : "v"(v3));
        asm("v_pk_add_f32 %0, %0, %1" : "+v"(d[4][q]) : "v"(v4));
        asm("v_pk_add_f32 %0, %0, %1" : "+v"(d[5][q]) : "v"(v5));
        wino4_bt6(d[0][q], d[1][q], d[2][q], d[3][q], d[4][q], d[5][q], k2, k4, k5);
    };
#elif defined(P4_ABL_PREVADD)
    auto pass_v = [&](int q) __attribute__((always_inline)) {
        const int qi = q == 0 ? 0 : q <= 2 ? 1 : q <= 4 ? 2 : 3;
        asm("v_pk_add_f32 %0, %0, %1" : "+v"(d[0][q]) : "v"(pv[0][qi]));
        asm("v_pk_add_f32 %0, %0, %1" : "+v"(d[1][q]) : "v"(pv[1][qi]));
        asm("v_pk_add_f32 %0, %0, %1" : "+v"(d[2][q]) : "v"(pv[1][qi]));
        asm("v_pk_add_f32 %0, %0, %1" : "+v"(d[3][q]) : "v"(pv[2][qi]));
        asm("v_pk_add_f32 %0, %0, %1" : "+v"(d[4][q]) : "v"(pv[2][qi]));
        asm("v_pk_add_f32 %0, %0, %1" : "+v"(d[5][q]) : "v"(pv[3][qi]));
        wino4_bt6(d[0][q], d[1][q], d[2][q], d[3][q], d[4][q], d[5][q], k2, k4, k5);
    };
#else
    auto pass_v = [&](int q) __attribute__((always_inline)) { wino4_bt6(d[0][q], d[1][q], d[2][q], d[3][q], d[4][q], d[5][q], k2, k4, k5); };
#endif
    auto pass_h = [&](int r) __attribute__((always_inline)) { wino4_bt6(d[r][0], d[r][1], d[r][2], d[r][3], d[r][4], d[r][5], k2, k4, k5); };
    auto write_row = [&](int buf, int r) __attribute__((always_inline)) {
#pragma unroll
        for (int b = 0; b < 6; ++b) *reinterpret_cast<f32x2*>(lds + buf * V_FLOATS + (r * 6 + b) * NT * CB + vw) = d[r][b];
    };

    Item w = decode(item);
    {
        const __amdgpu_buffer_rsrc_t r0 = make_rsrc(in_base(w.g, mine(w)));
#pragma unroll
        for (int k = 0; k < 36; ++k) issue(r0, 0, k / 6, k % 6);
    }
#pragma unroll
    for (int q = 0; q < 6; ++q) pass_v(q);
#pragma unroll
    for (int r = 0; r < 6; ++r) {
        pass_h(r);
        write_row(0, r);
    }
    {
        const bool one = (nchunk == 1);
        const Item w1 = (one && item + ISTEP < item_end) ? decode(item + ISTEP) : w;
        const __amdgpu_buffer_rsrc_t r1 = make_rsrc(in_base(w1.g, mine(w1)));
#pragma unroll
        for (int k = 0; k < 16; ++k) issue(r1, one ? 0 : PLANE_BYTES, 1 + k / 4, 1 + k % 4);
    }
    int vbuf = 0;
    __syncthreads();
    __amdgpu_buffer_rsrc_t rw = make_rsrc(w_base(w));
    f32x4 wq[RING];
#pragma unroll
    for (int dd = 0; dd < PRE; ++dd) wq[dd] = buf_load<P4_WAUX>(rw, wlane, dd * 1024);
    f32x4 bnext;
    auto load_bias = [&](const Item& wi) {
        const float* bias = p.bias + wi.g * p.bias_gs + wi.cb * 64 + 16 * a;
        const __amdgpu_buffer_rsrc_t rb = __builtin_amdgcn_make_buffer_rsrc(const_cast<float*>(bias), 0, 64, 0x00020000);
        bnext = buf_load<P4_WAUX>(rb, (unsigned)(fresh_lane() >> 4) * 16u, 0);
    };
    load_bias(w);

    for (;;) {
        f32x4 acc[NPOS][2];
        const bool more_items = item + ISTEP < item_end;
        const Item wnx = more_items ? decode(item + ISTEP) : w;
        const __amdgpu_buffer_rsrc_t rw_nx = more_items ? make_rsrc(w_base(wnx)) : rw;
        const char* in_cur = in_base(w.g, mine(w));
        const char* in_nx = in_base(wnx.g, mine(wnx));
        const bool more2 = item + 2 * ISTEP < item_end;
        const Item wn2 = (nchunk == 1 && more2) ? decode(item + 2 * ISTEP) : wnx;
        const char* in_n2 = in_base(wn2.g, mine(wn2));
        auto in_nx2 = [&](int over) { return (nchunk == 1 && over >= 1) ? in_n2 : in_nx; };
        acc[BIAS_XI][0] = bnext;
        acc[BIAS_XI][1] = bnext;
#ifdef P4_PROF
        const bool prof_on = (blockIdx.x == P4_PROF) && a == P4_PROF_WAVE && (item == prof_item);
#define P4_STAMP(row, col) do { if (prof_on && lane == 0) reinterpret_cast<unsigned long long*>(lds + 2 * V_FLOATS)[(row) * 40 + (col)] = __builtin_readcyclecounter(); } while (0)
#else
#define P4_STAMP(row, col) do { } while (0)
#endif

        auto chunk = [&](auto first_tag, int ch) __attribute__((always_inline)) {
            constexpr bool FIRST = decltype(first_tag)::value;
            const bool last_ch = (ch == nchunk - 1);
            const __amdgpu_buffer_rsrc_t r_stage = make_rsrc(last_ch ? in_nx : in_cur);
            const int stage_off = (last_ch ? 0 : ch + 1) * PLANE_BYTES;
            const bool wrap2 = ch + 2 >= nchunk;
            const __amdgpu_buffer_rsrc_t r_stage2 = make_rsrc(wrap2 ? in_nx2(ch + 2 - nchunk) : in_cur);
            const int stage_off2 = (wrap2 ? (ch + 2 - nchunk) % nchunk : ch + 2) * PLANE_BYTES;
            const int wcur_off = ch * CHUNK_W_BYTES;
            const __amdgpu_buffer_rsrc_t rw_over = last_ch ? rw_nx : rw;
            const int wover_off = last_ch ? 0 : (ch + 1) * CHUNK_W_BYTES;
            const float* vsrc = lds + vbuf * V_FLOATS + vr;
            const int wbuf = vbuf ^ 1;

            f32x4 bb[2][2];
            bb[0][0] = *reinterpret_cast<const f32x4*>(vsrc);
            bb[0][1] = *reinterpret_cast<const f32x4*>(vsrc + 16 * CB);
            static_for<0, NS>([&](auto Q) __attribute__((always_inline)) {
                constexpr int q = decltype(Q)::value;
                constexpr int xi = q;
                constexpr bool AG = xi < NPOS_A;
#ifdef P4_PROF
                if (ch < 15) P4_STAMP(ch, q);
#endif
#if P4_ILV
                {
                    const f32x4 av = wq[q % RING];
                    const f32x4 b0 = bb[q & 1][0], b1 = bb[q & 1][1];
                    constexpr bool ZR = FIRST && xi != BIAS_XI;
                    __builtin_amdgcn_sched_barrier(0);
                    mfma_pair<AG, ZR>(acc[xi][0], acc[xi][1], av[0], b0[0], b1[0]);
                    __builtin_amdgcn_sched_barrier(0);
#ifndef P4_ABL_NOWLOAD
                if constexpr (q % WB == 0) {
#pragma unroll
                    for (int dd = q + WD; dd < q + WD + WB; ++dd) {
                        if (FIRST && dd < PRE) continue;
                        if (dd < NS) wq[dd % RING] = buf_load<P4_WAUX>(rw, wlane, wcur_off + dd * 1024);
                        else wq[(dd - NS) % RING] = buf_load<P4_WAUX>(rw_over, wlane, wover_off + (dd - NS) * 1024);
                    }
                }
#endif
                    __builtin_amdgcn_sched_barrier(0);
                    mfma_pair<AG, false>(acc[xi][0], acc[xi][1], av[1], b0[1], b1[1]);
                    __builtin_amdgcn_sched_barrier(0);
                if constexpr (q + 1 < NS) {
                    bb[(q + 1) & 1][0] = *reinterpret_cast<const f32x4*>(vsrc + (q + 1) * NT * CB);
                    bb[(q + 1) & 1][1] = *reinterpret_cast<const f32x4*>(vsrc + (q + 1) * NT * CB + 16 * CB);
                }
                    __builtin_amdgcn_sched_barrier(0);
                    mfma_pair<AG, false>(acc[xi][0], acc[xi][1], av[2], b0[2], b1[2]);
                    __builtin_amdgcn_sched_barrier(0);
#if P4_ILV == 3
                if constexpr (q > TQ + 7 && q <= TQ + 13) write_row(wbuf, q - TQ - 8);
#endif
#ifndef P4_ABL_NOPATCH
                if constexpr (q >= HQ && q < HQ + 10) {
                    issue(r_stage, stage_off, halo_r(2 * (q - HQ)), halo_q(2 * (q - HQ)));
                    issue(r_stage, stage_off, halo_r(2 * (q - HQ) + 1), halo_q(2 * (q - HQ) + 1));
                }
#endif
#ifndef P4_ABL_NOPATCH
                if constexpr (q >= TQ + 9 && q <= TQ + 12) {
#pragma unroll
                    for (int u = 1; u <= 4; ++u) issue(r_stage2, stage_off2, q - TQ - 8, u);
                }
#endif
                    __builtin_amdgcn_sched_barrier(0);
                    mfma_pair<AG, false>(acc[xi][0], acc[xi][1], av[3], b0[3], b1[3]);
                    __builtin_amdgcn_sched_barrier(0);
#ifndef P4_ABL_NOXF
                if constexpr (q > TQ && q <= TQ + 6) pass_v(q - TQ - 1);
                if constexpr (q > TQ + 6 && q <= TQ + 12) pass_h(q - TQ - 7);
#endif
#if defined(P4_ABL_VWRITE_FAKE)
                if constexpr (q > TQ + 6 && q <= TQ + 12) { if (p.N < 0) write_row(wbuf, q - TQ - 7); }
#elif !defined(P4_ABL_NOVWRITE)
                if constexpr (P4_ILV != 3 && q > TQ + 6 && q <= TQ + 12) write_row(wbuf, q - TQ - 7);
#endif
                }
#else
#ifndef P4_ABL_NOWLOAD
                if constexpr (q % WB == 0) {
#pragma unroll
                    for (int dd = q + WD; dd < q + WD + WB; ++dd) {
                        if (FIRST && dd < PRE) continue;
                        if (dd < NS) wq[dd % RING] = buf_load<P4_WAUX>(rw, wlane, wcur_off + dd * 1024);
                        else wq[(dd - NS) % RING] = buf_load<P4_WAUX>(rw_over, wlane, wover_off + (dd - NS) * 1024);
                    }
                }
#endif
                if constexpr (q + 1 < NS) {
                    bb[(q + 1) & 1][0] = *reinterpret_cast<const f32x4*>(vsrc + (q + 1) * NT * CB);
                    bb[(q + 1) & 1][1] = *reinterpret_cast<const f32x4*>(vsrc + (q + 1) * NT * CB + 16 * CB);
                }
#ifdef P4_ABL_LDSPATCH
                if constexpr (q < P4_ABL_LDSPATCH) {
                    const unsigned voff = (unsigned)(q * 4096 + tid * 16);
                    asm volatile("s_mov_b32 m0, %2\n\tbuffer_load_dwordx4 %0, %1, 0 offen lds" ::"v"(voff), "s"(r_stage), "s"((unsigned)(LDS_BYTES + ((q & 3) * 4 + a) * 1024)) : "memory");
                }
#endif
#ifndef P4_ABL_NOPATCH
                if constexpr (q >= HQ && q < HQ + 10) {
                    issue(r_stage, stage_off, halo_r(2 * (q - HQ)), halo_q(2 * (q - HQ)));
                    issue(r_stage, stage_off, halo_r(2 * (q - HQ) + 1), halo_q(2 * (q - HQ) + 1));
                }
#endif
#ifndef P4_ABL_NOXF
                if constexpr (q > TQ && q <= TQ + 6) pass_v(q - TQ - 1);
                if constexpr (q > TQ + 6 && q <= TQ + 12) pass_h(q - TQ - 7);
#endif
#if defined(P4_ABL_VWRITE_FAKE)
                if constexpr (q > TQ + 6 && q <= TQ + 12) { if (p.N < 0) write_row(wbuf, q - TQ - 7); }
#elif !defined(P4_ABL_NOVWRITE)
                if constexpr (q > TQ + 6 && q <= TQ + 12) write_row(wbuf, q - TQ - 7);
#endif
#ifndef P4_ABL_NOPATCH
                if constexpr (q >= TQ + 9 && q <= TQ + 12) {
#pragma unroll
                    for (int u = 1; u <= 4; ++u) issue(r_stage2, stage_off2, q - TQ - 8, u);
                }
#endif
                __builtin_amdgcn_sched_barrier(0);
                const f32x4 av = wq[q % RING];
                const f32x4 b0 = bb[q & 1][0], b1 = bb[q & 1][1];
                mfma_step<AG, FIRST && xi != BIAS_XI>(acc[xi][0], acc[xi][1], av, b0, b1);
#endif
                __builtin_amdgcn_sched_barrier(0);
            });
#ifndef P4_ABL_NOBAR
            __syncthreads();
#endif
            vbuf ^= 1;
        };
        chunk(std::true_type{}, 0);
        for (int ch = 1; ch < nchunk; ++ch) chunk(std::false_type{}, ch);

#pragma unroll
        for (int dd = WD; dd < PRE; ++dd) wq[dd % RING] = buf_load<P4_WAUX>(rw_nx, wlane, dd * 1024);
        load_bias(wnx);
        P4_STAMP(15, 0);
        wait_mfma_results();
#ifdef P4_ABL_NOOUT
        if (acc[0][0][0] == 1.2345e-30f)
#endif
        {
            int relu_s = p.relu;
            asm volatile("" : "+s"(relu_s));
            const float floor_ = __builtin_bit_cast(float, __builtin_amdgcn_readfirstlane(relu_s ? 0 : (int)0xff7fffff));
            const int lane_o = fresh_lane();
            const int m_o = lane_o & 15;
            const unsigned olane = (unsigned)(m_o * 64 + (lane_o >> 4) * 16);
#pragma unroll
            for (int tb = 0; tb < 2; ++tb) {
                const Blk bo = tb ? w.b1 : w.b0;
                if (tb == 1 && w.nvalid == 1) continue;
                const int by_abs = bo.by + p.ty_off, bx_abs = bo.bx + p.tx_off;
                const long long origin = p.out_gs * w.g + ((((long long)bo.n * p.pl_byp + by_abs + 1) * p.pl_bxp + bx_abs + 1) * nplane_o + w.cb * 4 + a) * (long long)(PLANE_BYTES / 4);
                const __amdgpu_buffer_rsrc_t r_out = __builtin_amdgcn_make_buffer_rsrc(p.out + origin, 0, PLANE_BYTES, 0x00020000);
                const bool partial = (by_abs * BLK + BLK > p.Ho) || (bx_abs * BLK + BLK > p.Wo);
                f32x4 T[4][6];
#pragma unroll
                for (int b = 0; b < 6; ++b) {
                    const f32x4 m0 = acc[0 * 6 + b][tb], m1 = acc[1 * 6 + b][tb], m2 = acc[2 * 6 + b][tb], m3 = acc[3 * 6 + b][tb],
                                m4 = acc[4 * 6 + b][tb], m5 = acc[5 * 6 + b][tb];
#ifdef P4_ABL_NOVPASS
                    T[0][b] = m0; T[1][b] = m1 + m5; T[2][b] = m2 + m3; T[3][b] = m4;
#else
                    const f32x4 s1 = m1 + m2, d1 = sub4(m1, m2), s2 = m3 + m4, d2 = sub4(m3, m4);
                    T[0][b] = m0 + s1 + s2;
                    T[1][b] = d1 + 2.f * d2;
                    T[2][b] = s1 + 4.f * s2;
                    T[3][b] = (d1 + 8.f * d2) + m5;
#endif
                }
                const int rem_y = p.Ho - by_abs * BLK - 4 * (m_o >> 2), rem_x = p.Wo - bx_abs * BLK - 4 * (m_o & 3);
#pragma unroll
                for (int i = 0; i < 4; ++i) {
                    const f32x4 s1 = T[i][1] + T[i][2], d1 = sub4(T[i][1], T[i][2]), s2 = T[i][3] + T[i][4], d2 = sub4(T[i][3], T[i][4]);
                    f32x4 y[4];
                    y[0] = T[i][0] + s1 + s2;
                    y[1] = d1 + 2.f * d2;
                    y[2] = s1 + 4.f * s2;
                    y[3] = (d1 + 8.f * d2) + T[i][5];
#pragma unroll
                    for (int j = 0; j < 4; ++j) {
                        f32x4 o = y[j];
                        o[0] = fmaxf(o[0], floor_);
                        o[1] = fmaxf(o[1], floor_);
                        o[2] = fmaxf(o[2], floor_);
                        o[3] = fmaxf(o[3], floor_);
#ifdef P4_ABL_STOREOOB
                        const unsigned vo = 0x80000000u | olane;
#else
                        const unsigned vo = (!partial || (i < rem_y && j < rem_x)) ? olane : 0x80000000u;
#endif
#ifndef P4_ABL_NOSTORE
                        buf_store(o, r_out, vo, (i * 4 + j) * 1024);
#else
                        if (o[0] == 1.2345e-30f) buf_store(o, r_out, vo, (i * 4 + j) * 1024);
#endif
                    }
                }
            }
        }
#ifdef P4_PROF
        P4_STAMP(15, 1);
        if (prof_on) {
            __builtin_amdgcn_s_waitcnt(0);
            P4_STAMP(15, 2);
            __builtin_amdgcn_s_waitcnt(0);
            for (int i = lane; i < 16 * 40; i += 64) p4_prof_buf[i] = reinterpret_cast<unsigned long long*>(lds + 2 * V_FLOATS)[i];
        }
#endif
        if (!more_items) break;
        item += ISTEP;
        w = wnx;
        rw = rw_nx;
    }
}

hipError_t cerb_launch_wino4p(ConvParams p, hipStream_t st) {
    if (p.Cin % CB || p.Cout % 64 || p.resid || p.pl_byp < 3 || p.pl_bxp < 3 || p.H != p.Ho || p.W != p.Wo) return hipErrorInvalidValue;
    const long long nblk = wino4_block_grid(p);
    if (p.pl_byp != (p.Ho + BLK - 1) / BLK + 2 || p.pl_bxp != (p.Wo + BLK - 1) / BLK + 2) return hipErrorInvalidValue;
    const long long items = (long long)p.groups * ((nblk + 1) / 2) * (p.Cout / 64);
    const int tag = p.level_tag == 2 ? 2 : p.level_tag ? 1 : 0;
    auto kern = tag == 2 ? conv_wino4p_kernel<2> : tag ? conv_wino4p_kernel<1> : conv_wino4p_kernel<0>;
    static bool attr_done[3][64] = {};
    return wino4_launch(kern, attr_done[tag], items, LDS_BYTES + PROF_BYTES, p, st);
}

#ifdef P4_PROF
extern "C" int cerb_w4p_prof_read(unsigned long long* dst) { return (int)hipMemcpyFromSymbol(dst, HIP_SYMBOL(p4_prof_buf), sizeof(unsigned long long) * 16 * 40); }
#endif
```

### cerberus_amd/csrc/dev_entry.hip

```cpp
#include "cerb_net.h"

#define DEV_NEED(cond) \
    do {               \
        if (!(cond)) return (int)hipErrorInvalidValue; \
    } while (0)

extern "C" {

int cerb_dev_wgrad_wino_supported(int H, int W, int Cin, int Cout) { return cerb_wgrad_wino_supported(H, W, Cin, Cout) ? 1 : 0; }
size_t cerb_dev_wgrad_wino_workspace_bytes(int G, int N, int H, int W, int Cin, int Cout) {
    return cerb_wgrad_wino_supported(H, W, Cin, Cout) ? cerb_wgrad_wino_workspace_bytes(G, N, H, W, Cin, Cout) : 0;
}
int cerb_dev_wgrad_wino(const float* x, const float* dy, float* dw, float* db, int G, int N, int H, int W, int Cin, int Cout, long long x_gs, void* ws, void* st) {
    DEV_NEED(x && dy && dw && ws && G > 0 && N > 0);
    return (int)cerb_launch_wgrad_wino(x, dy, dw, G, N, H, W, Cin, Cout, x_gs, ws, (hipStream_t)st, db);
}

size_t cerb_dev_wgrad_workspace_bytes(int G, int N, int Ho, int Wo, int Cin, int Cout, int ks, int* slices_out) {
    return cerb_wgrad_workspace_bytes(G, N, Ho, Wo, Cin, Cout, ks, slices_out);
}
int cerb_dev_wgrad(const float* x, const float* dy, float* dw, float* db, int G, int N, int H, int W, int Cin, int Cout, int ks, int stride, long long x_gs, void* ws,
                   void* st) {
    DEV_NEED(x && dy && dw && ws && G > 0 && N > 0 && H > 0 && W > 0);
    return (int)cerb_launch_wgrad(x, dy, dw, G, N, H, W, Cin, Cout, ks, stride, x_gs, ws, (hipStream_t)st, db);
}

size_t cerb_dev_stem_wgrad_mfma_workspace_bytes() { return cerb_stem_wgrad_workspace_bytes(); }
int cerb_dev_stem_wgrad_mfma(const unsigned char* tiles, const float* dy, float* dw, int N, int H, int W, void* ws, void* st) {
    DEV_NEED(tiles && dy && dw && ws && N > 0 && H > 0 && W > 0);
    return (int)cerb_launch_stem_wgrad_mfma(tiles, dy, dw, N, H, W, ws, (hipStream_t)st);
}
int cerb_dev_stem_wgrad(const unsigned char* tiles, const float* dy, float* dw, int N, int H, int W, void* st) {
    DEV_NEED(tiles && dy && dw && N > 0 && H > 0 && W > 0);
    return (int)cerb_launch_stem_wgrad(tiles, dy, dw, N, H, W, (hipStream_t)st);
}

int cerb_dev_conv_bwd(const float* x, const float* dy, const float* w, float* dx, float* dw, float* db, int G, int N, int H, int W, int Cin, int Cout, int ks, int stride,
                      long long x_gs, void* st) {
    DEV_NEED(dy && (dx || dw || db) && (!dx || w) && (!dw || x) && G > 0 && N > 0 && (ks == 1 || ks == 3) && (stride == 1 || stride == 2));
    return (int)cerb_launch_conv_bwd(x, dy, w, dx, dw, db, G, N, H, W, Cin, Cout, ks, stride, x_gs, (hipStream_t)st);
}

size_t cerb_dev_bn_workspace_bytes(int groups, long long rows, int C) { return cerb_bn_workspace_bytes(groups, rows, C); }
size_t cerb_dev_bn_fold_workspace_bytes(int groups, int C) { return cerb_bn_fold_workspace_bytes(groups, C); }
int cerb_dev_bn_stats(const float* x, long long group_stride, long long rows, int C, int groups, float eps, float* mean, float* rstd, float* var_unbiased, void* ws,
                      void* st) {
    DEV_NEED(x && mean && rstd && ws && rows > 0 && groups > 0);
    return (int)cerb_launch_bn_stats(x, group_stride, rows, C, groups, eps, mean, rstd, var_unbiased, ws, (hipStream_t)st);
}
int cerb_dev_bn_finalize(const double* partial, int blocks, long long rows, int C, float eps, float* mean, float* rstd, float* var_unbiased, int groups, void* fold_ws,
                         void* st) {
    DEV_NEED(partial && mean && rstd && blocks > 0 && rows > 0 && groups > 0);
    return (int)cerb_launch_bn_finalize(partial, blocks, rows, C, eps, mean, rstd, var_unbiased, (hipStream_t)st, groups, fold_ws);
}
int cerb_dev_bn_bwd(const float* dz, const float* z, const float* y, float* dy, float* dresid, long long group_stride, long long rows, int C, int groups, const float* mean,
                    const float* rstd, const float* gamma, const float* beta, float* dgamma, float* dbeta, int relu, int dy_assign, int dresid_assign,
                    unsigned long long eval_mask, void* ws, void* st) {
    DEV_NEED(dz && y && dy && mean && rstd && gamma && dgamma && dbeta && ws && rows > 0 && groups > 0 && (!relu || z || (beta && !dresid)));
    return (int)cerb_launch_bn_bwd(dz, z, y, dy, dresid, group_stride, rows, C, groups, mean, rstd, gamma, beta, dgamma, dbeta, relu, dy_assign, ws, (hipStream_t)st, eval_mask,
                                   dresid_assign);
}

int cerb_dev_upadd_bwd_fused_ok(int H, int W, int C, int G) { return cerb_upadd_bwd_fused_ok(H, W, C, G) ? 1 : 0; }
int cerb_dev_upadd_bwd(const float* dout, float* dskip, float* dprev, int G, int N, int H, int W, int C, long long prev_gs, int shared_prev, unsigned group_mask,
                       int skip_assign, int prev_assign, void* st) {
    DEV_NEED(dout && dskip && dprev && G > 0 && N > 0 && H > 0 && W > 0 && H % 2 == 0 && W % 2 == 0 && C % 4 == 0);
    return (int)cerb_launch_upadd_bwd(dout, dskip, dprev, G, N, H, W, C, prev_gs, shared_prev, (hipStream_t)st, group_mask, skip_assign, prev_assign);
}

int cerb_dev_maxpool_idx(const float* in, float* out, unsigned* idx, int N, int H, int W, int C, void* st) {
    DEV_NEED(in && out && idx && N > 0 && H > 0 && W > 0 && C % 4 == 0);
    return (int)cerb_launch_maxpool_idx(in, out, idx, N, H, W, C, (hipStream_t)st);
}
int cerb_dev_maxpool_bwd_idx(const unsigned* idx, const float* dy, float* dx, int N, int H, int W, int C, void* st) {
    DEV_NEED(idx && dy && dx && N > 0 && H > 0 && W > 0 && H % 2 == 0 && W % 2 == 0 && C % 4 == 0);
    return (int)cerb_launch_maxpool_bwd_idx(idx, dy, dx, N, H, W, C, (hipStream_t)st);
}
int cerb_dev_maxpool_bwd(const float* x, const float* ypool, const float* dy, float* dx, int N, int H, int W, int C, void* st) {
    DEV_NEED(x && ypool && dy && dx && N > 0 && H > 0 && W > 0 && H % 2 == 0 && W % 2 == 0 && C % 4 == 0);
    return (int)cerb_launch_maxpool_bwd(x, ypool, dy, dx, N, H, W, C, (hipStream_t)st);
}

int cerb_dev_pointwise_bwd(const float* x, const float* dy, const float* w, float* dx, float* dw, float* db, long long rows, int cin, int cout, const float* in_scale,
                           int dx_assign, void* st) {
    DEV_NEED(dy && (dx || dw || db) && (!dx || w) && (!dw || x) && rows > 0 && cin > 0 && cout > 0);
    return (int)cerb_launch_pointwise_bwd(x, dy, w, dx, dw, db, rows, cin, cout, in_scale, dx_assign, (hipStream_t)st);
}
size_t cerb_dev_pw_bwd_small_workspace_bytes(long long rows, int cin, int cout) { return cerb_pw_bwd_small_workspace_bytes(rows, cin, cout); }
int cerb_dev_pw_bwd_small(const float* x, const float* dy, const float* w, float* dx, float* dw, float* db, long long rows, int cin, int cout, int dx_assign, void* ws,
                          void* st) {
    DEV_NEED(x && dy && w && ws && rows > 0 && cin > 0 && cout > 0);
    return (int)cerb_launch_pw_bwd_small(x, dy, w, dx, dw, db, rows, cin, cout, dx_assign, ws, (hipStream_t)st);
}
size_t cerb_dev_pw_wgrad_small_workspace_bytes(long long rows, int cin, int cout) { return cerb_pw_wgrad_small_workspace_bytes(rows, cin, cout); }
int cerb_dev_pw_wgrad_small(const float* x, const float* dy, float* dw, long long rows, int cin, int cout, void* ws, void* st) {
    DEV_NEED(x && dy && dw && ws && rows > 0 && cin > 0 && cout > 0);
    return (int)cerb_launch_pw_wgrad_small(x, dy, dw, rows, cin, cout, ws, (hipStream_t)st);
}

size_t cerb_dev_colsum_workspace_bytes(int C, int G) { return (size_t)G * 2048 * C * 4; }
int cerb_dev_colsum(const float* d, long long group_stride, long long rows, int C, int G, float* out, void* ws, void* st) {
    DEV_NEED(d && out && ws && rows > 0 && C > 0 && G > 0);
    return (int)cerb_launch_colsum(d, group_stride, rows, C, G, out, ws, (hipStream_t)st);
}
int cerb_dev_crop_gap(const float* x, int N, int H, int W, int C, int y0, int ch, int x0, int cw, float* out, void* st) {
    DEV_NEED(x && out && N > 0 && C > 0 && y0 >= 0 && x0 >= 0 && ch > 0 && cw > 0 && y0 + ch <= H && x0 + cw <= W);
    return (int)cerb_launch_crop_gap(x, N, H, W, C, y0, ch, x0, cw, out, (hipStream_t)st);
}
int cerb_dev_crop_gap_bwd(const float* dg, float* dx, int N, int H, int W, int C, int y0, int ch, int x0, int cw, void* st) {
    DEV_NEED(dg && dx && N > 0 && C > 0 && y0 >= 0 && x0 >= 0 && ch > 0 && cw > 0 && y0 + ch <= H && x0 + cw <= W);
    return (int)cerb_launch_crop_gap_bwd(dg, dx, N, H, W, C, y0, ch, x0, cw, (hipStream_t)st);
}
int cerb_dev_dilate2(const float* dy, float* d, long long n, int H, int W, int C, void* st) {
    DEV_NEED(dy && d && n > 0 && H > 0 && W > 0);
    return (int)cerb_launch_dilate2(dy, d, n, H, W, C, (hipStream_t)st);
}

long long cerb_devfwd_planar_elems(int N, int H, int W, int C) { return cerb_planar_elems(N, H, W, C); }
int cerb_devfwd_upsample2_add(const float* skip, const float* prev, float* out, int G, int N, int H, int W, int C, long long prev_gs, void* st) {
    DEV_NEED(skip && prev && out && G > 0 && N > 0 && H > 0 && W > 0 && H % 2 == 0 && W % 2 == 0 && C % 4 == 0);
    return (int)cerb_launch_upsample2_add(skip, prev, out, G, N, H, W, C, prev_gs, nullptr, (hipStream_t)st);
}
int cerb_devfwd_upsample2_add_planar(const float* skip, const float* prev, float* out, int G, int N, int H, int W, int C, long long prev_gs, long long out_gs,
                                     int prev_planar, void* st) {
    DEV_NEED(skip && prev && out && G > 0 && N > 0 && H > 0 && W > 0 && out_gs >= cerb_planar_elems(N, H, W, C));
    return (int)cerb_launch_upsample2_add_planar(skip, prev, out, G, N, H, W, C, prev_gs, out_gs, nullptr, prev_planar, (hipStream_t)st);
}

}
```

### cerberus_amd/csrc/net_kernels.hip

```cpp
#include "cerb_common.h"

struct StemParams {
    const unsigned char* tiles;
    const float* tiles_f32;
    const float* wpack;
    const float* bias;
    float* out;
    int N, H, W, tiles_x, tiles_y;
    int relu;
};

template <bool F32IN>
__global__ __launch_bounds__(256, 2) void stem_conv7x7_kernel(StemParams p) {
    constexpr int TH = 8, TW = 32, IH = TH + 6, IW = TW + 6, ROW = 120;
    __shared__ __attribute__((aligned(16))) float wl[7 * 12 * 2 * 64];
    __shared__ __attribute__((aligned(16))) float xl[IH * ROW];
    const int tid = threadIdx.x, lane = tid & 63, wave = tid >> 6, j = lane & 31, h = lane >> 5;
    for (int i = tid; i < 7 * 12 * 2 * 64; i += 256) wl[i] = p.wpack[i];
    const int ntile = p.N * p.tiles_y * p.tiles_x;
    for (int tile = blockIdx.x; tile < ntile; tile += gridDim.x) {
        int t_ = tile;
        const int tx = t_ % p.tiles_x;
        t_ /= p.tiles_x;
        const int ty = t_ % p.tiles_y;
// ... 174 lines not shown
        r /= bn_cnt;
        const int bm = (int)(r % bm_cnt) + bm_lo;
        const int n = (int)(r / bm_cnt);
        const int m0 = max(bm, 0), m1 = min(bm + 1, Hp - 1), n0 = max(bn, 0), n1 = min(bn + 1, Wp - 1);
        f32x4 sk[2][2];
        bool ok[2][2];
        long long o[2][2];
#pragma unroll
        for (int dy = 0; dy < 2; ++dy)
#pragma unroll
            for (int dx = 0; dx < 2; ++dx) {
                const int y = 2 * bm + 1 + dy, x = 2 * bn + 1 + dx;
                ok[dy][dx] = y >= 0 && y < H && x >= 0 && x < W;
                o[dy][dx] = (((long long)n * H + y) * W + x) * C + c4 * 4;
                if (ok[dy][dx]) sk[dy][dx] = *reinterpret_cast<const f32x4*>(skip + o[dy][dx]);
            }
        const long long pb = (long long)n * Hp * Wp * C + c4 * 4;
        for (int g = 0; g < groups; ++g) {
            const float* pg = prev + g * prev_gs + pb;
            const f32x4 p00 = *reinterpret_cast<const f32x4*>(pg + ((long long)m0 * Wp + n0) * C);
            const f32x4 p01 = *reinterpret_cast<const f32x4*>(pg + ((long long)m0 * Wp + n1) * C);
            const f32x4 p10 = *reinterpret_cast<const f32x4*>(pg + ((long long)m1 * Wp + n0) * C);
            const f32x4 p11 = *reinterpret_cast<const f32x4*>(pg + ((long long)m1 * Wp + n1) * C);
            const f32x4 top_l = blend2(0.75f, p00, 0.25f, p01), top_r = blend2(0.25f, p00, 0.75f, p01);
            const f32x4 bot_l = blend2(0.75f, p10, 0.25f, p11), bot_r = blend2(0.25f, p10, 0.75f, p11);
            const f32x4 u[2][2] = {{blend2(0.75f, top_l, 0.25f, bot_l), blend2(0.75f, top_r, 0.25f, bot_r)},
                                   {blend2(0.25f, top_l, 0.75f, bot_l), blend2(0.25f, top_r, 0.75f, bot_r)}};
#pragma unroll
            for (int dy = 0; dy < 2; ++dy)
#pragma unroll
                for (int dx = 0; dx < 2; ++dx)
                    if (ok[dy][dx]) __builtin_nontemporal_store(sk[dy][dx] + u[dy][dx], reinterpret_cast<f32x4*>(out + g * out_gs + o[dy][dx]));
        }
    }
}

hipError_t cerb_launch_upsample2_add(const float* skip, const float* prev, float* out, int groups, int N, int H, int W, int C,
                                     long long prev_gs, const int* roi, hipStream_t st) {
    int bm_lo = -1, bm_hi = H / 2 - 1, bn_lo = -1, bn_hi = W / 2 - 1;
    if (roi && roi[1] > roi[0] && roi[3] > roi[2]) {
        auto lo = [](int v) { return (v - 2 >= 0 ? (v - 2) / 2 : -1); };
        bm_lo = lo(roi[0]);
        bn_lo = lo(roi[2]);
        if ((roi[1] - 1) / 2 < bm_hi) bm_hi = (roi[1] - 1) / 2;
        if ((roi[3] - 1) / 2 < bn_hi) bn_hi = (roi[3] - 1) / 2;
    }
    const int bm_cnt = bm_hi - bm_lo + 1, bn_cnt = bn_hi - bn_lo + 1;
    const long long total = (long long)N * bm_cnt * bn_cnt * (C / 4);
    long long blocks = (total + 255) / 256;
    if (blocks > 256 * 32) blocks = 256 * 32;
    if (blocks < 1) blocks = 1;
    hipLaunchKernelGGL(upsample2_add_kernel, dim3((unsigned)blocks), dim3(256), 0, st, skip, prev, out, groups, N, H, W, C, prev_gs, bm_lo, bm_cnt, bn_lo,
                       bn_cnt);
    return hipGetLastError();
}

template <bool PREV_PLANAR, int C>
__global__ __launch_bounds__(256) void upsample2_add_planar_kernel(const float* __restrict__ skip, const float* __restrict__ prev, float* __restrict__ out,
                                                                   int groups, int N, int H, int W, long long prev_gs, long long out_gs, int byp, int bxp,
                                                                   int by_lo, int by_cnt, int bx_lo, int bx_cnt) {
    static_assert(C % 64 == 0, "four 16-channel planes per pass");
    constexpr int NCC = C / 16, NPASS = NCC / 4;
    const int Hp = H >> 1, Wp = W >> 1;
    const int lane = threadIdx.x & 63, m = lane >> 2, cq = lane & 3, ty = m >> 2, tx = m & 3;
    const int nwork = N * by_cnt * bx_cnt * NPASS;
    for (int wk = blockIdx.x; wk < nwork; wk += gridDim.x) {
        const int blk = wk / NPASS, cc = (wk % NPASS) * 4 + (int)(threadIdx.x >> 6);
        const int bx = blk % bx_cnt + bx_lo;
        const int r_ = blk / bx_cnt;
        const int by = r_ % by_cnt + by_lo, n = r_ / by_cnt;
        const int y0 = 16 * by + 4 * ty, x0 = 16 * bx + 4 * tx;
        if (y0 >= H || x0 >= W) continue;
        const int ch = cc * 16 + cq * 4;
        f32x4 sk[4][4];
#pragma unroll
        for (int i = 0; i < 4; ++i)
#pragma unroll
            for (int j = 0; j < 4; ++j) sk[i][j] = *reinterpret_cast<const f32x4*>(skip + (((long long)n * H + y0 + i) * W + x0 + j) * C + ch);
        int rr[4], qq[4];
#pragma unroll
        for (int k = 0; k < 4; ++k) {
            rr[k] = min(max((y0 >> 1) - 1 + k, 0), Hp - 1);
            qq[k] = min(max((x0 >> 1) - 1 + k, 0), Wp - 1);
        }
        float* ob = out + ((((long long)n * byp + by + 1) * bxp + bx + 1) * NCC + cc) * 4096 + lane * 4;
        long long pcol[4];
        if constexpr (PREV_PLANAR) {
#pragma unroll
            for (int k = 0; k < 4; ++k) pcol[k] = (long long)((qq[k] >> 4) + 1) * NCC * 4096 + ((qq[k] & 3) * 16 + ((qq[k] >> 2) & 3)) * 16;
        }
        const int pbyp = cerb_planar_blocks(Hp), pbxp = cerb_planar_blocks(Wp);
        for (int g = 0; g < groups; ++g) {
            const float* pg = PREV_PLANAR ? prev + g * prev_gs + (long long)cc * 4096 + cq * 4 : prev + g * prev_gs + (long long)n * Hp * Wp * C + ch;
            f32x4 h[4][4];
#pragma unroll
            for (int k = 0; k < 4; ++k) {
                f32x4 p0, p1, p2, p3;
                if constexpr (PREV_PLANAR) {
                    const float* pr = pg + (((long long)n * pbyp + (rr[k] >> 4) + 1) * pbxp) * NCC * 4096 + (((rr[k] & 3) << 2) * 16 + (((rr[k] >> 2) & 3) << 2)) * 16;
                    p0 = *reinterpret_cast<const f32x4*>(pr + pcol[0]); p1 = *reinterpret_cast<const f32x4*>(pr + pcol[1]);
                    p2 = *reinterpret_cast<const f32x4*>(pr + pcol[2]); p3 = *reinterpret_cast<const f32x4*>(pr + pcol[3]);
                } else {
                    const float* pr = pg + (long long)rr[k] * Wp * C;
                    p0 = *reinterpret_cast<const f32x4*>(pr + (long long)qq[0] * C); p1 = *reinterpret_cast<const f32x4*>(pr + (long long)qq[1] * C);
                    p2 = *reinterpret_cast<const f32x4*>(pr + (long long)qq[2] * C); p3 = *reinterpret_cast<const f32x4*>(pr + (long long)qq[3] * C);
                }
                h[k][0] = blend2(0.25f, p0, 0.75f, p1);
                h[k][1] = blend2(0.75f, p1, 0.25f, p2);
                h[k][2] = blend2(0.25f, p1, 0.75f, p2);
                h[k][3] = blend2(0.75f, p2, 0.25f, p3);
            }
            float* og = ob + g * out_gs;
#pragma unroll
            for (int j = 0; j < 4; ++j) {
                const f32x4 u0 = blend2(0.25f, h[0][j], 0.75f, h[1][j]), u1 = blend2(0.75f, h[1][j], 0.25f, h[2][j]), u2 = blend2(0.25f, h[1][j], 0.75f, h[2][j]),
                            u3 = blend2(0.75f, h[2][j], 0.25f, h[3][j]);
#ifndef UPP_PLAIN_STORE
                __builtin_nontemporal_store(sk[0][j] + u0, reinterpret_cast<f32x4*>(og + (0 * 4 + j) * 256));
                __builtin_nontemporal_store(sk[1][j] + u1, reinterpret_cast<f32x4*>(og + (1 * 4 + j) * 256));
                __builtin_nontemporal_store(sk[2][j] + u2, reinterpret_cast<f32x4*>(og + (2 * 4 + j) * 256));
                __builtin_nontemporal_store(sk[3][j] + u3, reinterpret_cast<f32x4*>(og + (3 * 4 + j) * 256));
#else
                *reinterpret_cast<f32x4*>(og + (0 * 4 + j) * 256) = sk[0][j] + u0;
                *reinterpret_cast<f32x4*>(og + (1 * 4 + j) * 256) = sk[1][j] + u1;
                *reinterpret_cast<f32x4*>(og + (2 * 4 + j) * 256) = sk[2][j] + u2;
                *reinterpret_cast<f32x4*>(og + (3 * 4 + j) * 256) = sk[3][j] + u3;
#endif
            }
        }
    }
}

hipError_t cerb_launch_upsample2_add_planar(const float* skip, const float* prev, float* out, int groups, int N, int H, int W, int C, long long prev_gs,
                                            long long out_gs, const int* roi, int prev_planar, hipStream_t st) {
    if ((C != 64 && C != 128 && C != 256) || (H & 3) || (W & 3)) return hipErrorInvalidValue;
    int by_lo = 0, by_hi = (H + 15) / 16, bx_lo = 0, bx_hi = (W + 15) / 16;
    if (roi && roi[1] > roi[0] && roi[3] > roi[2]) {
        by_lo = roi[0] / 16; by_hi = (roi[1] + 15) / 16;
        bx_lo = roi[2] / 16; bx_hi = (roi[3] + 15) / 16;
    }
    const long long nblk = (long long)N * (by_hi - by_lo) * (bx_hi - bx_lo);
    if (nblk <= 0 || nblk >= (1ll << 31)) return hipErrorInvalidValue;
#ifndef UPP_GRID
#define UPP_GRID 16
#endif
    const long long nwork = nblk * (C / 64);
    if (nwork >= (1ll << 31)) return hipErrorInvalidValue;
    long long blocks = nwork < 256 * UPP_GRID ? nwork : 256 * UPP_GRID;
    auto kern = C == 64    ? (prev_planar ? upsample2_add_planar_kernel<true, 64> : upsample2_add_planar_kernel<false, 64>)
                : C == 128 ? (prev_planar ? upsample2_add_planar_kernel<true, 128> : upsample2_add_planar_kernel<false, 128>)
                           : (prev_planar ? upsample2_add_planar_kernel<true, 256> : upsample2_add_planar_kernel<false, 256>);
    hipLaunchKernelGGL(kern, dim3((unsigned)blocks), dim3(256), 0, st, skip, prev, out, groups, N, H, W, prev_gs, out_gs,
                       cerb_planar_blocks(H), cerb_planar_blocks(W), by_lo, by_hi - by_lo, bx_lo, bx_hi - bx_lo);
    return hipGetLastError();
}

#ifndef HEAD_TPW
#define HEAD_TPW 2
#endif
typedef float f32x4h __attribute__((ext_vector_type(4)));
__device__ __forceinline__ void head_absmax_commit(unsigned int* word, float m) {
#pragma unroll
    for (int o = 32; o >= 1; o >>= 1) m = fmaxf(m, __shfl_xor(m, o));
    if ((threadIdx.x & 63) == 0) {
        const unsigned int b = __float_as_uint(m);
        if (b > __atomic_load_n(word, __ATOMIC_RELAXED)) atomicMax(word, b);
    }
}

template <bool ROI>
__global__ __launch_bounds__(256, 2) void head_kernel(HeadParams p) {
    const int tid = threadIdx.x, lane = tid & 63, px = lane & 15, ks = lane >> 4;
    const f32x4h* w1v = reinterpret_cast<const f32x4h*>(p.w1p) + lane;
    const f32x4h* w2v = reinterpret_cast<const f32x4h*>(p.w2p) + lane;
    struct BPos {
        int n, row, xb;
    };
    auto inc = [&](BPos b) {
        if (++b.xb == p.nxb) {
            b.xb = 0;
            if (++b.row == p.rows) {
                b.row = 0;
                ++b.n;
            }
        }
        return b;
    };
    const long long npix = (long long)p.N * p.H * p.W;
    long long pbase = ((long long)blockIdx.x * 4 + (tid >> 6)) * (64 * HEAD_TPW);
    BPos cur[4], nxt[4];
    if constexpr (ROI) {
        const int wave = __builtin_amdgcn_readfirstlane(tid >> 6);
        const unsigned nblk = (unsigned)p.N * (unsigned)p.rows * (unsigned)p.nxb;
        const unsigned b0 = ((unsigned)blockIdx.x * 4u + (unsigned)wave) * (4u * HEAD_TPW);
        const unsigned bc = b0 < nblk ? b0 : nblk;
        const unsigned r = bc / (unsigned)p.nxb;
        cur[0].xb = (int)(bc - r * (unsigned)p.nxb);
        cur[0].n = (int)(r / (unsigned)p.rows);
        cur[0].row = (int)(r - (unsigned)cur[0].n * (unsigned)p.rows);
#pragma unroll
        for (int pb = 1; pb < 4; ++pb) cur[pb] = inc(cur[pb - 1]);
        nxt[0] = inc(cur[3]);
#pragma unroll
        for (int pb = 1; pb < 4; ++pb) nxt[pb] = inc(nxt[pb - 1]);
    }
    auto ptr_of = [&](const BPos& b) {
        const int n = min(b.n, p.N - 1), x = min(p.xa0 + 16 * b.xb + px, p.W - 1);
        return p.feat + (((long long)n * p.H + p.row0 + b.row) * p.W + x) * 64 + 4 * ks;
    };
    auto feat_ptr = [&](int pb, bool next) {
        if constexpr (ROI) return ptr_of(next ? nxt[pb] : cur[pb]);
        const long long P = pbase + (next ? 64 : 0) + pb * 16 + px;
        return p.feat + (P < npix ? P : npix - 1) * 64 + 4 * ks;
    };
    f32x4h x[4];
#pragma unroll
    for (int pb = 0; pb < 4; ++pb) x[pb] = *reinterpret_cast<const f32x4h*>(feat_ptr(pb, false));
    float amax = 0.f;
#pragma unroll 1
    for (int task = 0; task < HEAD_TPW; ++task, pbase += 64) {
    f32x4h acc1[6][4];
#pragma unroll
    for (int blk = 0; blk < 6; ++blk) {
        const f32x4h bb = *reinterpret_cast<const f32x4h*>(p.b1 + blk * 16 + ks * 4);
#pragma unroll
        for (int pb = 0; pb < 4; ++pb) acc1[blk][pb] = bb;
    }
    const float* xp[4];
#pragma unroll
    for (int pb = 0; pb < 4; ++pb) xp[pb] = feat_ptr(pb, false);
#pragma unroll
    for (int g = 0; g < 4; ++g) {
        f32x4h xn[4];
        if (g + 1 < 4) {
#pragma unroll
            for (int pb = 0; pb < 4; ++pb) xn[pb] = *reinterpret_cast<const f32x4h*>(xp[pb] + (g + 1) * 16);
        } else if (task + 1 < HEAD_TPW) {
#pragma unroll
            for (int pb = 0; pb < 4; ++pb) xn[pb] = *reinterpret_cast<const f32x4h*>(feat_ptr(pb, true));
        }
#pragma unroll
        for (int blk = 0; blk < 6; ++blk) {
            const f32x4h a = w1v[(blk * 4 + g) * 64];
#pragma unroll
            for (int t = 0; t < 4; ++t)
#pragma unroll
                for (int pb = 0; pb < 4; ++pb) acc1[blk][pb] = __builtin_amdgcn_mfma_f32_16x16x4f32(a[t], x[pb][t], acc1[blk][pb], 0, 0, 0);
        }
        if (g + 1 < 4 || task + 1 < HEAD_TPW) {
#pragma unroll
            for (int pb = 0; pb < 4; ++pb) x[pb] = xn[pb];
        }
    }
#pragma unroll
    for (int blk = 0; blk < 6; ++blk)
#pragma unroll
        for (int pb = 0; pb < 4; ++pb)
#pragma unroll
            for (int r = 0; r < 4; ++r) acc1[blk][pb][r] = fmaxf(acc1[blk][pb][r], 0.f);
    f32x4h acc2[4];
    {
        const f32x4h b2 = *reinterpret_cast<const f32x4h*>(p.b2 + 4 * ks);
#pragma unroll
        for (int pb = 0; pb < 4; ++pb) acc2[pb] = b2;
    }
#pragma unroll
    for (int blk = 0; blk < 6; ++blk) {
        const f32x4h a = w2v[blk * 64];
#pragma unroll
        for (int r = 0; r < 4; ++r)
#pragma unroll
            for (int pb = 0; pb < 4; ++pb) acc2[pb] = __builtin_amdgcn_mfma_f32_16x16x4f32(a[r], acc1[blk][pb][r], acc2[pb], 0, 0, 0);
    }
    float lg[8];
#pragma unroll
    for (int e = 0; e < 4; ++e) {
        float lo = 0.f, hi = 0.f;
#pragma unroll
        for (int pb = 0; pb < 4; ++pb) {
            const float t0 = __shfl(acc2[pb][e], px), t1 = __shfl(acc2[pb][e], 16 + px);
            lo = (ks == pb) ? t0 : lo;
            hi = (ks == pb) ? t1 : hi;
        }
        lg[e] = lo;
        lg[4 + e] = hi;
    }
    int n, y_, x_;
    if constexpr (ROI) {
        int xb_ = cur[0].xb;
        n = cur[0].n;
        y_ = cur[0].row;
#pragma unroll
        for (int pb = 1; pb < 4; ++pb) {
            n = (ks == pb) ? cur[pb].n : n;
            y_ = (ks == pb) ? cur[pb].row : y_;
            xb_ = (ks == pb) ? cur[pb].xb : xb_;
        }
        y_ += p.row0;
        x_ = p.xa0 + 16 * xb_ + px;
#pragma unroll
        for (int pb = 0; pb < 4; ++pb) cur[pb] = nxt[pb];
        nxt[0] = inc(cur[3]);
#pragma unroll
        for (int pb = 1; pb < 4; ++pb) nxt[pb] = inc(nxt[pb - 1]);
        if (n >= p.N || x_ >= p.W) continue;
    } else {
// ... 485 lines not shown
```

### cerberus_amd/stream_bands.py

```python
import os
from collections import OrderedDict

import numpy as np
import torch

from .shard_postproc import BandState, _device_label_fn, _device_relabel_fn, _device_table_fn
from .wsi import SlideGeometry, WSIRunner, band_partition, downsample2_inst, half_size

LABEL_WS_BYTES_PX = 96
LABEL_BYTES_PX = 6
RESERVE_BYTES = 2 << 30
STREAM_HEADROOM = 0.10


def canvas_bytes_per_px(net):
    tot = inst = 0
    for _, hname, _, _ in net._decoders:
        b = 8 if hname == "INST" else 1 if hname == "TYPE" else 4
        tot += b
        inst += b if hname == "INST" else 0
    return tot, inst


def forward_workspace_bytes(batch, win):
    return int(0.40e9 * int(batch) * (int(win) / 256.0) ** 2) + int(0.4e9)


def hbm_budget(device=None):
    free = int(torch.cuda.mem_get_info(device)[0]) if torch.cuda.is_available() else 0
    if torch.cuda.is_available():
        free += max(0, int(torch.cuda.memory_reserved(device)) - int(torch.cuda.memory_allocated(device)))
        from . import _lib

        free += int(_lib.lib().cerb_device_bytes_held())
    cap = os.environ.get("CERB_HBM_BUDGET_GB")
    if cap and os.environ.get("CERB_HBM_BUDGET_FORCE", "0") == "1":
        return int(float(cap) * 1e9)
    return min(free, int(float(cap) * 1e9)) if cap else free


class SlidePlan(object):
    def __init__(self, **kw):
        self.__dict__.update(kw)

    def __repr__(self):
        return "SlidePlan(%s)" % ", ".join("%s=%r" % kv for kv in sorted(self.__dict__.items()))


def plan_slide(net, slide_hw, win, out, batch, rank=0, world=1, want_twin=True, max_band_px=None, margin=512, budget=None, allow_stream=True):
    geo = SlideGeometry(slide_hw, win, out)
    r0, r1 = geo.band(rank, world)
    cw = geo.cols * geo.out
    band_rows = (r1 - r0) * geo.out
    px = band_rows * cw
    cb_all, cb_inst = canvas_bytes_per_px(net)
    fwd = forward_workspace_bytes(batch, win)
    budget = hbm_budget() if budget is None else int(budget)
    y0, y1 = geo.input_rows(r0, r1)
    jpeg_ring = 0
    if os.environ.get("CERB_JPEG_DECODE") == "device":
        from .jpeg_device import ring_bytes_estimate

        jpeg_ring = ring_bytes_estimate(geo.W)
    slab = (y1 - y0) * geo.W * 3 + jpeg_ring
    halo = (2 * margin * cw) if world > 1 else 0
    call_px = min(px, int(max_band_px) if max_band_px else px) + 2 * margin * cw
    phase_infer = slab
    phase_label = px * LABEL_BYTES_PX + LABEL_WS_BYTES_PX * call_px + halo * (cb_inst + 4)
    resident = px * cb_all + max(phase_infer, phase_label) + fwd + RESERVE_BYTES
    if resident + (fwd if want_twin else 0) <= budget:
        return SlidePlan(mode="resident", sub_bands=1, twin=bool(want_twin), need=resident + (fwd if want_twin else 0), budget=budget)
    if resident <= budget:
        return SlidePlan(mode="resident", sub_bands=1, twin=False, need=resident, budget=budget)
    why = "rank %d of %d: a %d x %d px band needs %.1f GB resident (%.1f canvases, the larger of %.1f slab and %.1f labels + labelling workspace, %.1f forward workspace) of %.1f GB" % (
        rank, world, band_rows, cw, resident / 1e9, px * cb_all / 1e9, phase_infer / 1e9, phase_label / 1e9, fwd / 1e9, budget / 1e9)
    if allow_stream and any(hname == "INST" and int(och) == 2 for _, hname, och, _ in net._decoders):
        raise ValueError(why + "; a model with two-class INST heads (post-proc codes IP-ERODED-3 / IP-ERODED-11, --eroded_maps) is not streamed in "
                         "sub-bands: use more ranks, or a device with room for the resident band")
    if not allow_stream:
        return SlidePlan(mode="resident", sub_bands=1, twin=False, need=resident, budget=budget, over_budget=why + "; streaming is not available on this path: trying resident")
    rows = r1 - r0
    min_rows = max(1, -(-2 * margin // geo.out))
    tail = (-(-margin // geo.out)) * geo.out * cw * cb_all if world > 1 else 0
    best = tight = None
    for S in range(2, rows // min_rows + 1):
        rs = -(-rows // S)
        if rs < min_rows:
            break
        sub_px = rs * geo.out * cw
        sub_slab = (rs * geo.out + 2 * geo.ctx + 2) * geo.W * 3 + jpeg_ring
        strips = 2 * 3 * margin * cw * 8 + halo * (cb_inst + 4)
        need = sub_slab + 2 * sub_px * cb_all + tail + px * ((cb_all - cb_inst) + LABEL_BYTES_PX) + LABEL_WS_BYTES_PX * (sub_px + 2 * margin * cw) + 2 * sub_px * 4 + strips + fwd + RESERVE_BYTES
        best = need if best is None else min(best, need)
        if need <= budget and tight is None:
            tight = SlidePlan(mode="streamed", sub_bands=S, twin=False, need=need, budget=budget, resident_need=resident)
        if need <= budget * (1.0 - STREAM_HEADROOM):
            return SlidePlan(mode="streamed", sub_bands=S, twin=False, need=need, budget=budget, resident_need=resident)
    if tight is not None:
        return tight
    raise ValueError(why + "; streamed in sub-bands it still needs %.1f GB (class canvases + label maps stay resident: %.1f GB)" % (
        (best or 0) / 1e9, px * ((cb_all - cb_inst) + LABEL_BYTES_PX) / 1e9))


def agree_on_plan(plan, dist, dev):
    if dist is None:
        return plan
    t = torch.tensor([1 if plan.mode == "streamed" else 0], dtype=torch.int64, device=dev)
    dist.all_reduce(t, op=dist.ReduceOp.MAX)
    if int(t.item()) and plan.mode != "streamed":
        plan = SlidePlan(**dict(plan.__dict__, mode="streamed", sub_bands=1, twin=False, agreed="another rank streams"))
    return plan


def multi_ranks(world, dist):
    return dist is not None and int(world) > 1


def infer_and_label_streamed(net, source, slide_hw, win, out, batch, sub_bands, margin=512, guard=48, twin=None, label_fn=_device_label_fn,
                             table_fn=_device_table_fn, relabel_fn=_device_relabel_fn, prof=None, rank=0, world=1, dist=None, parts=None, watch=None,
                             arrays_fn=None, mask_fn=None):
    import time

    from .launch import null_watch
    from .postproc import mask_lumen_by_gland
    from .shard_postproc import _device_arrays_fn, _device_mask_fn, halo_exchange

    arrays_fn, mask_fn, watch = arrays_fn or _device_arrays_fn, mask_fn or _device_mask_fn, watch or null_watch()
    H, W = int(slide_hw[0]), int(slide_hw[1])
    geo = SlideGeometry((H, W), win, out)
    S = int(sub_bands)
    R0, R1 = geo.band(rank, world) if world > 1 else (0, geo.rows)
    cuts = [R0 + c for c in band_partition(R1 - R0, S)]
    assert out % 2 == 0 or not multi_ranks(world, dist), "sharded half-resolution maps need an even patch_output_shape"
    by0 = R0 * out
    bvalid = max(0, min((R1 - R0) * out, H - by0))
    multi = dist is not None and world > 1
    dev = torch.device("cuda", torch.cuda.current_device())
    tissues = [t for t in ("Nuclei", "Gland", "Lumen") if any(d[3] == t + "-INST" for d in net._decoders)]
    has_type = {t: any(d[3] == t + "-TYPE" for d in net._decoders) for t in tissues}
    small = OrderedDict()
    for _, hname, _, key in net._decoders:
        if hname != "INST":
            small[key] = torch.zeros((bvalid, W), dtype=torch.uint8 if hname == "TYPE" else torch.float32, device=dev)
    inst = OrderedDict()
    for t in tissues:
        inst[t] = torch.zeros((bvalid, W) if t == "Nuclei" else (half_size(bvalid), half_size(W)), dtype=torch.int32, device=dev)
    info = OrderedDict((t, {"n_owned": 0, "n_total": 0, "n_truncated": 0, "n_unresolved": 0, "local_bands": S, "streamed": True}) for t in tissues)
    pend = {t: None for t in tissues}
    down_above = {t: None for t in tissues}
    down_pend = {t: None for t in tissues}
    halo_below = {t: None for t in tissues}
    thalo = {t: [None, None] for t in tissues}
    pubs = {t: [] for t in tissues}
    last_pub = {t: np.zeros((0, 2), np.int64) for t in tissues}
    deferred = {t: [] for t in tissues}
    first_rows = {t: (0, 0) for t in tissues}
    local_parts = {t: [] for t in tissues}
    t_inf = t_lab = 0.0

    def mt(t, half):
        m = margin.get(t, margin.get("default", 512)) if isinstance(margin, dict) else margin
        return (m // 2, guard // 2) if half else (m, guard)

    def type_rows(t, half):
        tm = small[t + "-TYPE"]
        return tm[::2, ::2][: inst[t].shape[0], : inst[t].shape[1]] if half else tm

    def type_window(st, t, half):
        ty0 = by0 // 2 if half else by0
        tm = type_rows(t, half)
        g0 = st.y0 - st.top - ty0
        g1 = g0 + st.h_win
        pieces = []
        if g0 < 0:
            pieces.append(thalo[t][0][g0:] if g0 > -thalo[t][0].shape[0] else thalo[t][0])
        pieces.append(tm[max(g0, 0): min(g1, tm.shape[0])])
        if g1 > tm.shape[0]:
            pieces.append(thalo[t][1][: g1 - tm.shape[0]])
# ... 179 lines not shown
```

Measured before the change: 155.9.

## Run encoder stages in tile-planar layout with planar Winograd residual convs

Adds a tile-planar path for the first three ResNet encoder stages. Maxpool and the strided igemm convs now write directly into a blocked planar layout, the stride-1 convs use a new Winograd-planar kernel variant that fuses the residual add, and each stage is converted back to NHWC once at its end. The aim is cheaper, better-coalesced Winograd tile loads and stores in the encoder, which previously ran in NHWC. In exchange it allocates extra planar buffers (the workspace estimate is raised), adds a conversion pass per stage, and adds new template variants.

```diff
diff --git a/cerberus_amd/csrc/cerb_api.hip b/cerberus_amd/csrc/cerb_api.hip
--- a/cerberus_amd/csrc/cerb_api.hip
+++ b/cerberus_amd/csrc/cerb_api.hip
@@ -542,9 +542,11 @@
                                              "conv_wino4p<f4x4,16x16x2,planar,half-res>", "conv_wino4p<f4x4,16x16x2,planar>"};
 static const char* const kPlanarEntryFamily[4] = {"upsample2_add_planar<eighth-res>", "upsample2_add_planar<quarter-res>", "upsample2_add_planar", "upsample2_add_planar"};
 
+static constexpr int kEncPlanarStages = 0x7;
+
 int run_conv(cerb_net* net, const std::string& name, const float* in, const float* prev, const float* resid, float* out, int N,
              int H, int W, int relu, int mode, long long in_gs, long long prev_gs, hipStream_t st, double* macs,
-             const int* roi, long long planar_out_gs) {
+             const int* roi, long long planar_out_gs, int enc) {
     auto it = net->conv.find(name);
     if (it == net->conv.end()) return fail("internal: conv " + name + " not packed");
     const PackedConv& c = it->second;
@@ -574,13 +576,14 @@
     const double fl = 2.0 * (double)c.groups * N * p.Ho * p.Wo * (double)c.cout * c.cin * c.ks * c.ks;
     const long long map_px = (long long)p.Ho * p.Wo;
     const bool use_w4 = net->conv_algo == 5 || net->conv_algo == 7 || (net->conv_algo == 6 && map_px >= 256);
-    const bool planar = planar_out_gs > 0;
+    const bool planar = planar_out_gs > 0 && enc != 2;
     static const long long w4b_max_px = [] {
         const char* e = cerb_dev_getenv("CERB_W4B_MAX_PX");
         return e ? atoll(e) : 4096ll;
     }();
     const bool w4b = !planar && (net->conv_algo == 7 || (net->conv_algo == 6 && map_px <= w4b_max_px)) && c.cin % 64 == 0;
-    if (planar && !(use_w4 && c.wino && mode == 0 && net->fold_bn && !resid)) return fail("internal: conv " + name + " cannot take the planar path");
+    if (planar && !(use_w4 && c.wino && mode == 0 && net->fold_bn && (!resid || enc == 1))) return fail("internal: conv " + name + " cannot take the planar path");
+    if (enc == 2 && !(c.stride == 2 && mode == 0 && net->fold_bn && !resid && planar_out_gs > 0)) return fail("internal: conv " + name + " cannot store tile-planar");
     if (use_w4 && c.wino && mode == 0 && (!it->second.host_w.empty() || !net->fold_bn)) {
         PackedConv& cm = it->second;
         float* train_slot = nullptr;
@@ -606,11 +609,12 @@
         }
         if (planar) {
             p.out_gs = planar_out_gs;
-            p.level_tag = net->planar_level == 3 ? 1 : net->planar_level == 2 ? 0 : 2;
+            p.level_tag = enc ? 3 : net->planar_level == 3 ? 1 : net->planar_level == 2 ? 0 : 2;
             p.pl_byp = cerb_planar_blocks(p.Ho);
             p.pl_bxp = cerb_planar_blocks(p.Wo);
         }
-        if (prof_begin(net, name, planar ? kPlanarFamily[net->planar_level & 3] : w4b ? (cerb_wino4b_packed(p) ? (resid ? "conv_wino4b<f4x4,16t,res>" : "conv_wino4b<f4x4,16t>") : (resid ? "conv_wino4b<f4x4,16x16,res>" : "conv_wino4b<f4x4,16x16>")) : (resid ? "conv_wino4<f4x4,16x16x2,res>" : "conv_wino4<f4x4,16x16x2>"), fl_done, st)) return 1;
+        const std::string enc_family = enc ? "conv_wino4_enc_planar<f4x4,16x16x2," + std::to_string(p.Ho) + (p.Ho == p.Wo ? "^2" : "x" + std::to_string(p.Wo)) + (resid ? ",res>" : ">") : std::string();
+        if (prof_begin(net, name, enc ? enc_family.c_str() : planar ? kPlanarFamily[net->planar_level & 3] : w4b ? (cerb_wino4b_packed(p) ? (resid ? "conv_wino4b<f4x4,16t,res>" : "conv_wino4b<f4x4,16t>") : (resid ? "conv_wino4b<f4x4,16x16,res>" : "conv_wino4b<f4x4,16x16>")) : (resid ? "conv_wino4<f4x4,16x16x2,res>" : "conv_wino4<f4x4,16x16x2>"), fl_done, st)) return 1;
         if (net->conv_bn_part && !planar && !resid && !(roi && roi[1] > roi[0] && roi[3] > roi[2])) {
             p.bn_part = net->conv_bn_part;
             net->conv_bn_bpg = w4b ? cerb_wino4b_bn_blocks(p) : N * ((p.Ho + 15) / 16) * ((p.Wo + 15) / 16);
@@ -634,8 +638,13 @@
         if (prof_end(net, st)) return 1;
         return 0;
     }
+    if (enc == 2) {
+        p.out_gs = planar_out_gs;
+        p.pl_byp = cerb_planar_blocks(p.Ho);
+        p.pl_bxp = cerb_planar_blocks(p.Wo);
+    }
     const std::string kn = "conv_igemm<ks" + std::to_string(c.ks) + ",s" + std::to_string(c.stride) + ",mode" + std::to_string(mode) +
-                           (p.Wo < 32 ? ",16x16>" : ",8x32>");
+                           (p.Wo < 32 ? ",16x16" : ",8x32") + (enc == 2 ? ",planar>" : ">");
     if (prof_begin(net, name, kn, fl, st)) return 1;
     HIP_OK(cerb_launch_conv(p, c.ks, c.stride, mode, st));
     if (prof_end(net, st)) return 1;
@@ -670,13 +679,38 @@
         }
         return true;
     };
+    const int enc_mask = [] {
+        const char* e = cerb_dev_getenv("CERB_ENC_PLANAR");
+        return e ? atoi(e) : kEncPlanarStages;
+    }();
+    auto stage_geometry_ok = [&](int li) {
+        if (dry || !net->planar || !net->fold_bn || net->conv_algo != 6 || !((enc_mask >> li) & 1)) return false;
+        const int h = hs[li + 1], w = ws[li + 1];
+        if (h < 16 || w < 16 || (h & 15) || (w & 15)) return false;
+        for (int b = 0; b < kLayers[li]; ++b)
+            for (int j = 1; j <= 2; ++j) {
+                auto c = net->conv.find("backbone.layer" + std::to_string(li + 1) + "." + std::to_string(b) + ".conv" + std::to_string(j));
+                if (c == net->conv.end() || c->second.cout % 64 || c->second.cin % 16 || (c->second.stride == 1 && (!c->second.wino || c->second.host_w.empty()))) return false;
+            }
+        return true;
+    };
+    const bool enc_pl[4] = {stage_geometry_ok(0), stage_geometry_ok(1), stage_geometry_ok(2), stage_geometry_ok(3)};
+    auto stage_is_planar = [&](int li) { return enc_pl[li]; };
     if (!dry) {
-        if (net->x0.ensure((size_t)N * H * W * 64 * 4, guard) || net->pool.ensure((size_t)N * hs[1] * ws[1] * 64 * 4, guard)) return fail_alloc();
+        size_t need_t = 0, need_pool = stage_is_planar(0) ? 0 : (size_t)N * hs[1] * ws[1] * 64 * 4;
+        for (int li = 0; li < 4; ++li)
+            if (!stage_is_planar(li)) {
+                need_t = std::max(need_t, (size_t)N * hs[li + 1] * ws[li + 1] * kFilters[li + 1] * 4);
+                if (li > 0) need_pool = std::max(need_pool, (size_t)N * hs[li + 1] * ws[li + 1] * kFilters[li + 1] * 4);
+            }
+        if (net->x0.ensure((size_t)N * H * W * 64 * 4, guard) || net->pool.ensure(need_pool, guard)) return fail_alloc();
         for (int i = 1; i < 5; ++i)
             if (net->x[i].ensure((size_t)N * hs[i] * ws[i] * kFilters[i] * 4, guard)) return fail_alloc();
-        if (net->ta.ensure((size_t)N * hs[1] * ws[1] * 64 * 4, guard) || net->tb.ensure((size_t)N * hs[1] * ws[1] * 64 * 4, guard) ||
-            net->cm.ensure((size_t)N * hs[4] * ws[4] * 256 * 4, guard))
+        if (net->ta.ensure(need_t, guard) || net->tb.ensure(need_t, guard) || net->cm.ensure((size_t)N * hs[4] * ws[4] * 256 * 4, guard))
             return fail_alloc();
+        for (int li = 0; li < 4; ++li)
+            if (stage_is_planar(li) && (net->penc[li][0].ensure(1, N, hs[li + 1], ws[li + 1], kFilters[li + 1], st) || net->penc[li][1].ensure(1, N, hs[li + 1], ws[li + 1], kFilters[li + 1], st)))
+                return fail_alloc();
         if (D) {
             static const bool exact_ws = cerb_dev_getenv("CERB_LEGACY_WS") == nullptr;
             size_t need_sum = 0, need_mid = 0;
@@ -707,7 +741,8 @@
         HIP_OK(cerb_launch_stem(sp, st));
         if (prof_end(net, st)) return 1;
         if (prof_begin(net, "maxpool", "maxpool3x3s2", 0.0, st)) return 1;
-        HIP_OK(cerb_launch_maxpool(net->x0.p, net->pool.p, N, H, W, 64, st));
+        if (stage_is_planar(0)) HIP_OK(cerb_launch_maxpool_planar(net->x0.p, net->penc[0][0].b.p, N, H, W, 64, st));
+        else HIP_OK(cerb_launch_maxpool(net->x0.p, net->pool.p, N, H, W, 64, st));
         if (prof_end(net, st)) return 1;
     }
     float* cur = dry ? nullptr : net->pool.p;
@@ -715,6 +750,26 @@
     for (int li = 0; li < 4; ++li) {
         const int planes = kFilters[li + 1];
         const int Hi = (li == 0) ? hs[1] : hs[li], Wi = (li == 0) ? ws[1] : ws[li];
+        if (stage_is_planar(li)) {
+            PlanarBuf &bx = net->penc[li][0], &bt = net->penc[li][1];
+            const int ho = hs[li + 1], wo = ws[li + 1];
+            for (int b = 0; b < kLayers[li]; ++b) {
+                const std::string p = "backbone.layer" + std::to_string(li + 1) + "." + std::to_string(b);
+                if (b == 0 && li > 0) {
+                    if (run_conv(net, p + ".conv1", cur, nullptr, nullptr, bt.b.p, N, Hi, Wi, 1, 0, 0, 0, st, macs, nullptr, bt.gs(), 2)) return 1;
+                    if (run_conv(net, p + ".downsample", cur, nullptr, nullptr, bx.b.p, N, Hi, Wi, 0, 0, 0, 0, st, macs, nullptr, bx.gs(), 2)) return 1;
+                } else if (run_conv(net, p + ".conv1", bx.b.p, nullptr, nullptr, bt.b.p, N, ho, wo, 1, 0, bx.gs(), 0, st, macs, nullptr, bt.gs(), 1)) {
+                    return 1;
+                }
+                if (run_conv(net, p + ".conv2", bt.b.p, nullptr, bx.b.p, bx.b.p, N, ho, wo, 1, 0, bt.gs(), 0, st, macs, nullptr, bx.gs(), 1)) return 1;
+            }
+            if (prof_begin(net, "backbone.layer" + std::to_string(li + 1) + ".out", "planar_to_nhwc", 0.0, st)) return 1;
+            HIP_OK(cerb_launch_planar_to_nhwc(bx.b.p, net->x[li + 1].p, N, ho, wo, planes, st));
+            if (prof_end(net, st)) return 1;
+            cur = net->x[li + 1].p;
+            inpl = planes;
+            continue;
+        }
         for (int b = 0; b < kLayers[li]; ++b) {
             const std::string p = "backbone.layer" + std::to_string(li + 1) + "." + std::to_string(b);
             const int stride = (b == 0 && li > 0) ? 2 : 1;
diff --git a/cerberus_amd/csrc/cerb_net.h b/cerberus_amd/csrc/cerb_net.h
--- a/cerberus_amd/csrc/cerb_net.h
+++ b/cerberus_amd/csrc/cerb_net.h
@@ -108,6 +108,8 @@
                                  const float* dgamma, const float* dbeta, const float* w1, const float* w2, float* dprev, float* dw1, float* db1, long long rows, int out,
                                  int eval_mode, int assign, void* ws, hipStream_t st, const float* const* in_bn = nullptr, double* in_part = nullptr);
 hipError_t cerb_launch_maxpool(const float* in, float* out, int N, int H, int W, int C, hipStream_t st);
+hipError_t cerb_launch_maxpool_planar(const float* in, float* out, int N, int H, int W, int C, hipStream_t st);
+hipError_t cerb_launch_planar_to_nhwc(const float* in, float* out, int N, int H, int W, int C, hipStream_t st);
 hipError_t cerb_launch_head(const HeadParams& p, hipStream_t st);
 hipError_t cerb_launch_head_group(const HeadParams* heads, int n_heads, hipStream_t st, int w2_44);
 struct PatchClassParams {
@@ -263,6 +265,7 @@
     int planar_level = 3;
     PlanarBuf psum2, pmid2, pout2;
     PlanarBuf psum1, pmid1, pout1, psum0, pmid0, pout0;
+    PlanarBuf penc[4][2];
     int packed_items = 1;
     int planar = 1;
     bool profiling = false;
@@ -288,6 +291,7 @@
         if (copy_tab) (void)hipFree(copy_tab);
         if (pack_tab) (void)hipFree(pack_tab);
         x0.release(); pool.release(); ta.release(); tb.release(); cm.release(); dmid.release(); dsum.release(); psum.release(); pmid.release(); pout.release(); psum2.release(); pmid2.release(); pout2.release(); psum1.release(); pmid1.release(); pout1.release(); psum0.release(); pmid0.release(); pout0.release();
+        for (auto& s : penc) for (auto& b : s) b.release();
         t_mean.release(); t_rstd.release(); t_ws.release(); t_hid.release(); t_gap.release(); t_pc1.release(); t_idn.release(); t_dil.release();
         for (auto& b : tape) b.release();
         for (auto& b : x) b.release();
@@ -303,5 +307,5 @@
 int train_wino2_fresh(cerb_net* net, const std::string& name, PackedConv& cm, int dgrad, hipStream_t st);
 int train_wino4_slot(cerb_net* net, const std::string& name, PackedConv& cm, int w4b, int dgrad, hipStream_t st, float** out);
 int run_conv(cerb_net* net, const std::string& name, const float* in, const float* prev, const float* resid, float* out, int N, int H, int W, int relu, int mode,
-             long long in_gs, long long prev_gs, hipStream_t st, double* macs, const int* roi = nullptr, long long planar_out_gs = 0);
+             long long in_gs, long long prev_gs, hipStream_t st, double* macs, const int* roi = nullptr, long long planar_out_gs = 0, int enc = 0);
 #endif
diff --git a/cerberus_amd/csrc/conv_igemm.hip b/cerberus_amd/csrc/conv_igemm.hip
--- a/cerberus_amd/csrc/conv_igemm.hip
+++ b/cerberus_amd/csrc/conv_igemm.hip
@@ -40,7 +40,7 @@
     int g, cb, n, oy0, ox0, tx, ty;
 };
 
-template <int KS, int STRIDE, int TH, int TW, int CB, int MODE>
+template <int KS, int STRIDE, int TH, int TW, int CB, int MODE, bool PLANAR_OUT = false>
 __global__ __launch_bounds__(256, 2) void conv_igemm_kernel(ConvParams p) {
     using C = ConvCfg<KS, STRIDE, TH, TW, CB, MODE>;
     constexpr int WD = C::WD;
@@ -345,6 +345,15 @@
             const __amdgpu_buffer_rsrc_t r_res = make_rsrc(p.resid ? p.resid + w.g * p.resid_gs + origin : p.out);
             const bool has_res = p.resid != nullptr;
             const bool partial = (w.oy0 + TH > p.Ho) || (w.ox0 + TW > p.Wo);
+            [[maybe_unused]] const __amdgpu_buffer_rsrc_t r_pl = make_rsrc(p.out + w.g * p.out_gs + (long long)w.n * p.pl_byp * p.pl_bxp * (p.Cout >> 4) * 4096);
+            [[maybe_unused]] unsigned poffs[2] = {0u, 0u};
+            if constexpr (PLANAR_OUT) {
+#pragma unroll
+                for (int q = 0; q < 2; ++q) {
+                    const int pl = (wave * 2 + q) * 32 + j;
+                    poffs[q] = (unsigned)((cerb_planar_offset(0, w.oy0 + pl / TW, w.ox0 + pl % TW, w.cb * 4, p.pl_byp, p.pl_bxp, p.Cout >> 4) + 4 * h) * 4);
+                }
+            }
 #pragma unroll
             for (int q = 0; q < 2; ++q) {
                 if (partial) {
@@ -365,7 +374,8 @@
                             o[2] = fmaxf(o[2], 0.f);
                             o[3] = fmaxf(o[3], 0.f);
                         }
-                        buf_store(o, r_out, ooff[q], co * 4);
+                        if constexpr (PLANAR_OUT) buf_store(o, r_pl, poffs[q], (co >> 4) * 16384 + (co & 15) * 4);
+                        else buf_store(o, r_out, ooff[q], co * 4);
                     }
                 }
             }
@@ -377,13 +387,13 @@
     }
 }
 
-template <int KS, int STRIDE, int TH, int TW, int CB, int MODE>
+template <int KS, int STRIDE, int TH, int TW, int CB, int MODE, bool PLANAR_OUT = false>
 static hipError_t launch_cfg(ConvParams p, hipStream_t st) {
     using C = ConvCfg<KS, STRIDE, TH, TW, CB, MODE>;
     p.tiles_x = (p.Wo + TW - 1) / TW;
     p.tiles_y = (p.Ho + TH - 1) / TH;
     const long long items = (long long)p.groups * p.N * p.tiles_x * p.tiles_y * (p.Cout / 64);
-    auto kern = conv_igemm_kernel<KS, STRIDE, TH, TW, CB, MODE>;
+    auto kern = conv_igemm_kernel<KS, STRIDE, TH, TW, CB, MODE, PLANAR_OUT>;
     static bool attr_done[64] = {};
     if (cerb_attr_needed(attr_done)) {
         hipError_t e = hipFuncSetAttribute(reinterpret_cast<const void*>(kern), hipFuncAttributeMaxDynamicSharedMemorySize, C::LDS_BYTES);
@@ -402,6 +412,13 @@
 
 hipError_t cerb_launch_conv(const ConvParams& p, int ks, int stride, int mode, hipStream_t st) {
     const bool small = p.Wo < 32;
+    if (p.pl_byp > 0) {
+        if (mode != 0 || stride != 2 || p.resid || p.pl_byp != cerb_planar_blocks(p.Ho) || p.pl_bxp != cerb_planar_blocks(p.Wo) || p.Cout % 64) return hipErrorInvalidValue;
+        if ((long long)p.pl_byp * p.pl_bxp * (p.Cout / 16) * 16384 >= (1ll << 31)) return hipErrorInvalidValue;
+        if (ks == 3) return small ? launch_cfg<3, 2, 16, 16, 16, 0, true>(p, st) : launch_cfg<3, 2, 8, 32, 16, 0, true>(p, st);
+        if (ks == 1) return small ? launch_cfg<1, 2, 16, 16, 16, 0, true>(p, st) : launch_cfg<1, 2, 8, 32, 16, 0, true>(p, st);
+        return hipErrorInvalidValue;
+    }
     if (ks == 3 && stride == 1 && mode == 0) return small ? launch_cfg<3, 1, 16, 16, 32, 0>(p, st) : launch_cfg<3, 1, 8, 32, 32, 0>(p, st);
     if (ks == 3 && stride == 1 && mode == 1) return small ? launch_cfg<3, 1, 16, 16, 32, 1>(p, st) : launch_cfg<3, 1, 8, 32, 32, 1>(p, st);
     if (ks == 3 && stride == 2 && mode == 0) return small ? launch_cfg<3, 2, 16, 16, 16, 0>(p, st) : launch_cfg<3, 2, 8, 32, 16, 0>(p, st);
diff --git a/cerberus_amd/csrc/conv_wino4p.hip b/cerberus_amd/csrc/conv_wino4p.hip
--- a/cerberus_amd/csrc/conv_wino4p.hip
+++ b/cerberus_amd/csrc/conv_wino4p.hip
@@ -138,6 +138,7 @@
 template <int LEVEL>
 __global__ __launch_bounds__(256) __attribute__((amdgpu_waves_per_eu(1, 1))) void conv_wino4p_kernel(ConvParams p) {
     extern __shared__ __attribute__((aligned(16))) float lds[];
+    constexpr bool ENC = LEVEL == 4;
     const int tid = threadIdx.x;
     const int lane = tid & 63;
     const int a = __builtin_amdgcn_readfirstlane(tid >> 6);
@@ -170,7 +171,7 @@
     };
     auto decode = [&](int it) {
         Item w;
-        w.g = it / per_group;
+        w.g = ENC ? 0 : it / per_group;
         const int L = it - w.g * per_group;
         w.cb = L % ncb;
         const int pr = L / ncb;
@@ -183,11 +184,12 @@
 #ifdef P4_ABL_PATCHL2
         return reinterpret_cast<const char*>(p.in) + (((long long)(b.by & 1)) * p.pl_bxp + (b.bx & 3)) * (long long)nchunk * PLANE_BYTES;
 #endif
+        if constexpr (ENC) return reinterpret_cast<const char*>(p.in) + (((long long)b.n * p.pl_byp + b.by) * p.pl_bxp + b.bx) * (long long)nchunk * PLANE_BYTES;
         return reinterpret_cast<const char*>(p.in + g * p.in_gs) +
                (((long long)b.n * p.pl_byp + (b.by + p.ty_off)) * p.pl_bxp + (b.bx + p.tx_off)) * (long long)nchunk * PLANE_BYTES;
     };
     auto w_base = [&](const Item& w) {
-        return reinterpret_cast<const char*>(p.wpack + w.g * p.w_gs) + (long long)w.cb * nchunk * CHUNK_W_BYTES + a * WAVE_W_BYTES;
+        return reinterpret_cast<const char*>(p.wpack + (ENC ? 0 : w.g * p.w_gs)) + (long long)w.cb * nchunk * CHUNK_W_BYTES + a * WAVE_W_BYTES;
     };
 
     const int t = tid >> 3, c = tid & 7, tm = t & 15, tty = tm >> 2, ttx = tm & 3;
@@ -323,7 +325,7 @@
     for (int dd = 0; dd < PRE; ++dd) wq[dd] = buf_load<P4_WAUX>(rw, wlane, dd * 1024);
     f32x4 bnext;
     auto load_bias = [&](const Item& wi) {
-        const float* bias = p.bias + wi.g * p.bias_gs + wi.cb * 64 + 16 * a;
+        const float* bias = p.bias + (ENC ? 0 : wi.g * p.bias_gs) + wi.cb * 64 + 16 * a;
         const __amdgpu_buffer_rsrc_t rb = __builtin_amdgcn_make_buffer_rsrc(const_cast<float*>(bias), 0, 64, 0x00020000);
         bnext = buf_load<P4_WAUX>(rb, (unsigned)(fresh_lane() >> 4) * 16u, 0);
     };
@@ -501,14 +503,31 @@
             const int lane_o = fresh_lane();
             const int m_o = lane_o & 15;
             const unsigned olane = (unsigned)(m_o * 64 + (lane_o >> 4) * 16);
+#ifndef P4_RES_AHEAD
+#define P4_RES_AHEAD 1
+#endif
+            constexpr int RA = P4_RES_AHEAD;
+            [[maybe_unused]] f32x4 res[RA + 1][4];
 #pragma unroll
             for (int tb = 0; tb < 2; ++tb) {
                 const Blk bo = tb ? w.b1 : w.b0;
                 if (tb == 1 && w.nvalid == 1) continue;
-                const int by_abs = bo.by + p.ty_off, bx_abs = bo.bx + p.tx_off;
-                const long long origin = p.out_gs * w.g + ((((long long)bo.n * p.pl_byp + by_abs + 1) * p.pl_bxp + bx_abs + 1) * nplane_o + w.cb * 4 + a) * (long long)(PLANE_BYTES / 4);
+                const int by_abs = bo.by + (ENC ? 0 : p.ty_off), bx_abs = bo.bx + (ENC ? 0 : p.tx_off);
+                const long long blk_o = ((((long long)bo.n * p.pl_byp + by_abs + 1) * p.pl_bxp + bx_abs + 1) * nplane_o + w.cb * 4 + a) * (long long)(PLANE_BYTES / 4);
+                const long long origin = (ENC ? 0 : p.out_gs * w.g) + blk_o;
                 const __amdgpu_buffer_rsrc_t r_out = __builtin_amdgcn_make_buffer_rsrc(p.out + origin, 0, PLANE_BYTES, 0x00020000);
-                const bool partial = (by_abs * BLK + BLK > p.Ho) || (bx_abs * BLK + BLK > p.Wo);
+                const bool partial = !ENC && ((by_abs * BLK + BLK > p.Ho) || (bx_abs * BLK + BLK > p.Wo));
+                const int rem_y = p.Ho - by_abs * BLK - 4 * (m_o >> 2), rem_x = p.Wo - bx_abs * BLK - 4 * (m_o & 3);
+                [[maybe_unused]] auto res_request = [&](int i) __attribute__((always_inline)) {
+                    const __amdgpu_buffer_rsrc_t r_res = __builtin_amdgcn_make_buffer_rsrc(const_cast<float*>(p.resid + blk_o), 0, PLANE_BYTES, 0x00020000);
+#pragma unroll
+                    for (int j = 0; j < 4; ++j)
+                        res[i % (RA + 1)][j] = buf_load(r_res, (!partial || (i < rem_y && j < rem_x)) ? olane : 0x80000000u, (i * 4 + j) * 1024);
+                };
+                if constexpr (LEVEL == 4) {
+#pragma unroll
+                    for (int i = 0; i < RA; ++i) res_request(i);
+                }
                 f32x4 T[4][6];
 #pragma unroll
                 for (int b = 0; b < 6; ++b) {
@@ -524,7 +543,6 @@
                     T[3][b] = (d1 + 8.f * d2) + m5;
 #endif
                 }
-                const int rem_y = p.Ho - by_abs * BLK - 4 * (m_o >> 2), rem_x = p.Wo - bx_abs * BLK - 4 * (m_o & 3);
 #pragma unroll
                 for (int i = 0; i < 4; ++i) {
                     const f32x4 s1 = T[i][1] + T[i][2], d1 = sub4(T[i][1], T[i][2]), s2 = T[i][3] + T[i][4], d2 = sub4(T[i][3], T[i][4]);
@@ -533,6 +551,11 @@
                     y[1] = d1 + 2.f * d2;
                     y[2] = s1 + 4.f * s2;
                     y[3] = (d1 + 8.f * d2) + T[i][5];
+                    if constexpr (LEVEL == 4) {
+                        if (i + RA < 4) res_request(i + RA);
+#pragma unroll
+                        for (int j = 0; j < 4; ++j) y[j] = y[j] + res[i % (RA + 1)][j];
+                    }
 #pragma unroll
                     for (int j = 0; j < 4; ++j) {
                         f32x4 o = y[j];
@@ -571,13 +594,15 @@
 }
 
 hipError_t cerb_launch_wino4p(ConvParams p, hipStream_t st) {
-    if (p.Cin % CB || p.Cout % 64 || p.resid || p.pl_byp < 3 || p.pl_bxp < 3 || p.H != p.Ho || p.W != p.Wo) return hipErrorInvalidValue;
+    if (p.Cin % CB || p.Cout % 64 || p.pl_byp < 3 || p.pl_bxp < 3 || p.H != p.Ho || p.W != p.Wo) return hipErrorInvalidValue;
+    if (p.level_tag < 0 || p.level_tag > 3 || (p.resid && p.level_tag != 3)) return hipErrorInvalidValue;
     const long long nblk = wino4_block_grid(p);
+    if (p.level_tag == 3 && (p.groups != 1 || p.ty_off || p.tx_off || p.tiles_y * BLK != p.Ho || p.tiles_x * BLK != p.Wo)) return hipErrorInvalidValue;
     if (p.pl_byp != (p.Ho + BLK - 1) / BLK + 2 || p.pl_bxp != (p.Wo + BLK - 1) / BLK + 2) return hipErrorInvalidValue;
     const long long items = (long long)p.groups * ((nblk + 1) / 2) * (p.Cout / 64);
-    const int tag = p.level_tag == 2 ? 2 : p.level_tag ? 1 : 0;
-    auto kern = tag == 2 ? conv_wino4p_kernel<2> : tag ? conv_wino4p_kernel<1> : conv_wino4p_kernel<0>;
-    static bool attr_done[3][64] = {};
+    const int tag = p.resid ? 4 : p.level_tag;
+    auto kern = tag == 4 ? conv_wino4p_kernel<4> : tag == 3 ? conv_wino4p_kernel<3> : tag == 2 ? conv_wino4p_kernel<2> : tag ? conv_wino4p_kernel<1> : conv_wino4p_kernel<0>;
+    static bool attr_done[5][64] = {};
     return wino4_launch(kern, attr_done[tag], items, LDS_BYTES + PROF_BYTES, p, st);
 }
 
diff --git a/cerberus_amd/csrc/dev_entry.hip b/cerberus_amd/csrc/dev_entry.hip
--- a/cerberus_amd/csrc/dev_entry.hip
+++ b/cerberus_amd/csrc/dev_entry.hip
@@ -127,4 +127,40 @@
     return (int)cerb_launch_upsample2_add_planar(skip, prev, out, G, N, H, W, C, prev_gs, out_gs, nullptr, prev_planar, (hipStream_t)st);
 }
 
+int cerb_devfwd_maxpool(const float* in, float* out, int N, int H, int W, int C, int planar, void* st) {
+    DEV_NEED(in && out && N > 0 && H > 0 && W > 0 && C % 4 == 0);
+    return (int)(planar ? cerb_launch_maxpool_planar(in, out, N, H, W, C, (hipStream_t)st) : cerb_launch_maxpool(in, out, N, H, W, C, (hipStream_t)st));
 }
+int cerb_devfwd_planar_to_nhwc(const float* in, float* out, int N, int H, int W, int C, void* st) {
+    DEV_NEED(in && out);
+    return (int)cerb_launch_planar_to_nhwc(in, out, N, H, W, C, (hipStream_t)st);
+}
+int cerb_devfwd_conv(const float* in, const float* w_raw, float* wpack, const float* bias, const float* resid, float* out, int N, int H, int W, int Cin, int Cout, int ks,
+                     int stride, int relu, int kind, void* st) {
+    DEV_NEED(in && w_raw && wpack && bias && out && N > 0 && H > 0 && W > 0 && kind >= 0 && kind <= 3 && (ks == 1 || ks == 3) && (stride == 1 || stride == 2));
+    DEV_NEED(kind < 2 || (ks == 3 && stride == 1));
+    ConvParams p;
+    memset(&p, 0, sizeof(p));
+    p.in = in; p.wpack = wpack; p.bias = bias; p.resid = resid; p.out = out;
+    p.N = N; p.H = H; p.W = W; p.Cin = Cin; p.Cout = Cout;
+    p.Ho = stride == 2 ? H / 2 : H;
+    p.Wo = stride == 2 ? W / 2 : W;
+    p.relu = relu;
+    p.groups = 1;
+    p.bias_gs = Cout;
+    p.w_gs = (long long)Cout * Cin * (kind < 2 ? ks * ks : 36);
+    p.out_gs = (kind == 1 || kind == 3) ? cerb_planar_elems(N, p.Ho, p.Wo, Cout) : (long long)N * p.Ho * p.Wo * Cout;
+    if (kind == 1 || kind == 3) {
+        p.pl_byp = cerb_planar_blocks(p.Ho);
+        p.pl_bxp = cerb_planar_blocks(p.Wo);
+    }
+    hipError_t e = kind < 2 ? cerb_launch_pack_conv(w_raw, wpack, Cout, Cin, ks, cerb_conv_chunk(ks, stride), (hipStream_t)st)
+                            : cerb_launch_pack_wino4(w_raw, wpack, Cout, Cin, 0, kind == 2 ? 1 : 0, 1, (hipStream_t)st);
+    if (e != hipSuccess) return (int)e;
+    if (kind < 2) return (int)cerb_launch_conv(p, ks, stride, 0, (hipStream_t)st);
+    if (kind == 2) return (int)cerb_launch_wino4b(p, (hipStream_t)st);
+    p.level_tag = 3;
+    return (int)cerb_launch_wino4p(p, (hipStream_t)st);
+}
+
+}
diff --git a/cerberus_amd/csrc/net_kernels.hip b/cerberus_amd/csrc/net_kernels.hip
--- a/cerberus_amd/csrc/net_kernels.hip
+++ b/cerberus_amd/csrc/net_kernels.hip
@@ -350,6 +350,84 @@
                            : (prev_planar ? upsample2_add_planar_kernel<true, 256> : upsample2_add_planar_kernel<false, 256>);
     hipLaunchKernelGGL(kern, dim3((unsigned)blocks), dim3(256), 0, st, skip, prev, out, groups, N, H, W, prev_gs, out_gs,
                        cerb_planar_blocks(H), cerb_planar_blocks(W), by_lo, by_hi - by_lo, bx_lo, bx_hi - bx_lo);
+    return hipGetLastError();
+}
+
+__global__ __launch_bounds__(256) void maxpool3x3s2_kernel_planar(const float* __restrict__ in, float* __restrict__ out, int N, int H, int W, int C, int Ho, int Wo) {
+    const int byn = (Ho + 15) >> 4, bxn = (Wo + 15) >> 4, byp = byn + 2, bxp = bxn + 2, ncc = C >> 4, npass = C >> 6;
+    const int ty = threadIdx.x >> 6, tx = (threadIdx.x >> 4) & 3, q = threadIdx.x & 15;
+    const long long nwork = (long long)N * byn * bxn * npass * 16;
+    const long long per_xcd = gridDim.x / 8, vb = (long long)(blockIdx.x & 7) * per_xcd + (blockIdx.x >> 3);
+    for (long long wk = vb; wk < nwork; wk += gridDim.x) {
+        const int ij = (int)(wk & 15);
+        long long r = wk >> 4;
+        const int pass = (int)(r % npass);
+        r /= npass;
+        const int bx = (int)(r % bxn);
+        r /= bxn;
+        const int by = (int)(r % byn), n = (int)(r / byn);
+        const int cc = pass * 4 + (q >> 2), ch = cc * 16 + (q & 3) * 4;
+        const int oy = 16 * by + 4 * ty + (ij >> 2), ox = 16 * bx + 4 * tx + (ij & 3);
+        if (oy >= Ho || ox >= Wo) continue;
+        f32x4 m = {-INFINITY, -INFINITY, -INFINITY, -INFINITY};
+#pragma unroll
+        for (int ky = 0; ky < 3; ++ky) {
+            const int y = oy * 2 - 1 + ky;
+            if (y < 0 || y >= H) continue;
+#pragma unroll
+            for (int kx = 0; kx < 3; ++kx) {
+                const int x = ox * 2 - 1 + kx;
+                if (x < 0 || x >= W) continue;
+                const f32x4 v = *reinterpret_cast<const f32x4*>(in + (((long long)n * H + y) * W + x) * C + ch);
+                m[0] = fmaxf(m[0], v[0]);
+                m[1] = fmaxf(m[1], v[1]);
+                m[2] = fmaxf(m[2], v[2]);
+                m[3] = fmaxf(m[3], v[3]);
+            }
+        }
+        *reinterpret_cast<f32x4*>(out + ((((long long)n * byp + by + 1) * bxp + bx + 1) * ncc + cc) * 4096 + ij * 256 + (ty * 4 + tx) * 16 + (q & 3) * 4) = m;
+    }
+}
+
+hipError_t cerb_launch_maxpool_planar(const float* in, float* out, int N, int H, int W, int C, hipStream_t st) {
+    if (C % 64 || N <= 0 || H <= 0 || W <= 0) return hipErrorInvalidValue;
+    const int Ho = (H + 2 - 3) / 2 + 1, Wo = (W + 2 - 3) / 2 + 1;
+    const long long nwork = (long long)N * ((Ho + 15) / 16) * ((Wo + 15) / 16) * (C / 64) * 16;
+    long long blocks = (nwork + 7) / 8 * 8;
+    if (blocks > 256 * 64) blocks = 256 * 64;
+    hipLaunchKernelGGL(maxpool3x3s2_kernel_planar, dim3((unsigned)blocks), dim3(256), 0, st, in, out, N, H, W, C, Ho, Wo);
+    return hipGetLastError();
+}
+
+__global__ __launch_bounds__(256) void planar_to_nhwc_kernel(const float* __restrict__ in, float* __restrict__ out, int N, int H, int W, int C) {
+    const int byn = (H + 15) >> 4, bxn = (W + 15) >> 4, byp = byn + 2, bxp = bxn + 2, ncc = C >> 4, npass = C >> 6;
+    const int ty = threadIdx.x >> 6, tx = (threadIdx.x >> 4) & 3, q = threadIdx.x & 15;
+    const long long nwork = (long long)N * byn * bxn * npass;
+    for (long long wk = blockIdx.x; wk < nwork; wk += gridDim.x) {
+        const int pass = (int)(wk % npass);
+        long long r = wk / npass;
+        const int bx = (int)(r % bxn);
+        r /= bxn;
+        const int by = (int)(r % byn), n = (int)(r / byn);
+        const int cc = pass * 4 + (q >> 2), ch = cc * 16 + (q & 3) * 4;
+        const int y0 = 16 * by + 4 * ty, x0 = 16 * bx + 4 * tx;
+        const float* ib = in + ((((long long)n * byp + by + 1) * bxp + bx + 1) * ncc + cc) * 4096 + (ty * 4 + tx) * 16 + (q & 3) * 4;
+        f32x4 v[16];
+#pragma unroll
+        for (int ij = 0; ij < 16; ++ij) v[ij] = __builtin_nontemporal_load(reinterpret_cast<const f32x4*>(ib + ij * 256));
+#pragma unroll
+        for (int ij = 0; ij < 16; ++ij) {
+            const int y = y0 + (ij >> 2), x = x0 + (ij & 3);
+            if (y < H && x < W) *reinterpret_cast<f32x4*>(out + (((long long)n * H + y) * W + x) * C + ch) = v[ij];
+        }
+    }
+}
+
+hipError_t cerb_launch_planar_to_nhwc(const float* in, float* out, int N, int H, int W, int C, hipStream_t st) {
+    if (C % 64 || N <= 0 || H <= 0 || W <= 0) return hipErrorInvalidValue;
+    const long long nwork = (long long)N * ((H + 15) / 16) * ((W + 15) / 16) * (C / 64);
+    const long long blocks = nwork < 256 * 16 ? nwork : 256 * 16;
+    hipLaunchKernelGGL(planar_to_nhwc_kernel, dim3((unsigned)blocks), dim3(256), 0, st, in, out, N, H, W, C);
     return hipGetLastError();
 }
 
diff --git a/cerberus_amd/stream_bands.py b/cerberus_amd/stream_bands.py
--- a/cerberus_amd/stream_bands.py
+++ b/cerberus_amd/stream_bands.py
@@ -23,7 +23,7 @@
 
 
 def forward_workspace_bytes(batch, win):
-    return int(0.40e9 * int(batch) * (int(win) / 256.0) ** 2) + int(0.4e9)
+    return int(0.44e9 * int(batch) * (int(win) / 256.0) ** 2) + int(0.4e9)
 
 
 def hbm_budget(device=None):
```

New measurement: 157.1, median of 6. No clear change (+0.7%).
